# kisarur/minimap2-fpga

Measured on AMD Instinct MI355X. Metric: anchors/sec chained, higher is better.
Workload: dtype int32; 1 GPU; synthetic ONT anchor stream (mixed), 5000 anchors/read, map-ont chaining params (max_dist=5000, bw=500, max_iter=5000, max_skip=25), HBM-resident; reads_whole_batch=65536, distinct_reads=8192, anchors_per_read=5000, preset=map-ont, ragged=False, parallelism=read-sharded x1

## Files before the change

### include/mm2chain.h

```cpp
#ifndef MM2CHAIN_H
#define MM2CHAIN_H

#include <stdint.h>
#include <stddef.h>

#ifdef __cplusplus
extern "C" {
#endif

typedef struct { uint64_t x, y; } mm2c_anchor_t;

enum {
	MM2C_OK = 0,
	MM2C_E_NODEVICE = -1,
	MM2C_E_ARG = -2,
	MM2C_E_TOOBIG = -3,
	MM2C_E_HIP = -4
};

#define MM2C_F_IGNORE_SEG  0x1
#define MM2C_F_FORCE_GENERAL 0x2

typedef struct {
	int32_t max_dist_x, max_dist_y, bw;
// ... 13 lines not shown
int  mm2c_numa_cpulist(const char *sysfs_root, const char *pci_bus_id, char *buf, size_t len);
int  mm2c_slot_worker_node(int slot);
int  mm2c_split_tasks(int64_t n_tasks, const int64_t *offsets, int n_parts, int64_t *bounds );
void mm2c_shutdown(void);
const char *mm2c_last_error(void);
int  mm2c_device_info(char *name, size_t name_len, int *cu_count, size_t *hbm_bytes);
int  mm2c_device_identity(int *ordinal, char *pci_bus_id, size_t bus_len, char *arch, size_t arch_len);
int  mm2c_tune(const char *key, int value);

int  mm2c_split_model(const char *preset, float *k1_hw, float *k2_hw, float *c_hw, float *k_sw, float *c_sw);

void mm2c_params_map_ont(mm2c_params_t *p);
void mm2c_params_fpga_v2(mm2c_params_t *p, int32_t max_dist_x, int32_t max_dist_y, int32_t bw, int32_t q_span);

typedef struct mm2c_plan mm2c_plan_t;
mm2c_plan_t *mm2c_plan_create(const mm2c_params_t *par, int64_t n_tasks, const int64_t *h_offsets);
void mm2c_plan_destroy(mm2c_plan_t *plan);
int64_t mm2c_plan_total_anchors(const mm2c_plan_t *plan);

#define MM2C_STREAM_LIBRARY ((void *)(intptr_t)-1)

int mm2c_plan_run_device(mm2c_plan_t *plan, const void *d_anchors, const float *d_avg_qspan,
                         int32_t *d_f, int32_t *d_p, void *stream);

int mm2c_plan_set_device_offsets(mm2c_plan_t *plan, const int64_t *d_offsets);

int mm2c_plan_run_device_n(mm2c_plan_t *plan, const void *d_anchors, int64_t n_anchors, const float *d_avg_qspan, int64_t n_avg,
                           int32_t *d_f, int64_t n_f, int32_t *d_p, int64_t n_p, void *stream);

int mm2c_plan_last_kernel_ms(mm2c_plan_t *plan, float *ms);
int mm2c_plan_last_route(mm2c_plan_t *plan, int64_t *pieces, int64_t *one_wave_pieces, int64_t *coop_pieces);
int mm2c_route_pieces(int64_t pieces, int64_t longest, int64_t total);
int mm2c_plan_last_variant(mm2c_plan_t *plan, char *buf, size_t len);
int  mm2c_last_host_variant(char *buf, size_t len);
int  mm2c_debug_label_hits(unsigned long long *hits , int reset);
int mm2c_plan_last_prepass_ms(mm2c_plan_t *plan, float *ms);

int mm2c_plan_predict_device(mm2c_plan_t *plan, const void *d_anchors, uint8_t *d_num_subparts,
                             int64_t *d_total_subparts, int64_t *d_total_trip_count, void *stream);

int mm2c_chain_batch_host(const mm2c_params_t *par, int64_t n_tasks, const int64_t *h_offsets,
                          const mm2c_anchor_t *h_anchors, const float *h_avg_qspan ,
                          int32_t *h_f, int32_t *h_p);

void *mm2c_pinned_alloc(size_t bytes);
void  mm2c_pinned_free(void *ptr);

#define MM2C_MAX_TASK_ANCHORS ((int64_t)2147483582)

int mm2c_chain_task_host(const mm2c_params_t *par, int64_t n, const mm2c_anchor_t *a, float avg_qspan_scaled,
                         int32_t *f, int32_t *p, int tid);

int mm2c_chain_task_host_pred(const mm2c_params_t *par, int64_t n, const mm2c_anchor_t *a, float avg_qspan_scaled,
                              int32_t *f, int32_t *p, int tid, float hw_time_pred, float sw_time_pred);

typedef struct { int32_t device; int32_t reserved; uint64_t passes, calls, anchors, declined; } mm2c_slot_stats_t;
int mm2c_get_slot_stats(int slot, mm2c_slot_stats_t *out);
int mm2c_route_slot(int n_slots, const int64_t *outstanding, int tid);

#ifndef MM2C_NO_MM_CHAIN_DP_DECL
mm2c_anchor_t *mm_chain_dp(int max_dist_x, int max_dist_y, int bw, int max_skip, int max_iter, int min_cnt,
                           int min_sc, float gap_scale, int is_cdna, int n_segs, int64_t n, mm2c_anchor_t *a,
                           int *n_u_, uint64_t **_u, void *km, int tid);
#endif


// ... 164 lines not shown
```

### minimap2-fpga_amd/csrc/api_internal.h

```cpp
#ifndef MM2C_API_INTERNAL_H
#define MM2C_API_INTERNAL_H
#include <hip/hip_runtime.h>
#include <algorithm>
#include <atomic>
#include <chrono>
#include <condition_variable>
#include <cstdarg>
#include <cstdio>
#include <cstdlib>
#include <cstring>
#include <functional>
#include <thread>
#include <mutex>
#include <numeric>
#include <vector>
#include "mm2chain.h"
#include "chain_kernel.h"

namespace mm2c_api {

extern thread_local char g_err[512];
int fail(int code, const char *fmt, ...);

#define HIP_TRY(expr) do { hipError_t e_ = (expr); if (e_ != hipSuccess) \
	return ::mm2c_api::fail(MM2C_E_HIP, "%s failed: %s (%s:%d)", #expr, hipGetErrorString(e_), __FILE__, __LINE__); } while (0)

struct ThreadCtx;

struct Global {
	std::mutex mu;
	std::atomic<bool> ready{false};
	int device = -1;
	std::vector<int> devices;
	std::atomic<int64_t> multi_min_anchors{1 << 20};
	std::atomic<int> ring_class{3};
	std::atomic<int> far_thr10{7};
	std::atomic<int> noskip_loop{1};
	std::atomic<int> heap_sort{0};
	std::atomic<int> wide_pct{40};
	std::atomic<int> split_streams{1};
	std::atomic<int> compact_ring{1};
	std::atomic<int> q24_ring{1};
	std::atomic<int> force_tab{0};
	std::atomic<int> far_ring{1};
	std::atomic<int> epi_fused{1};
	std::atomic<size_t> combine_max_anchors{1u << 17};
	std::atomic<size_t> stage_max_anchors{1u << 21};
	std::atomic<int64_t> pipeline_chunk_anchors{20 << 20};
	std::atomic<int64_t> pipeline_pieces{8}, pipeline_min_chunk{4 << 20};
	std::atomic<int64_t> pipeline_taper{0};
	std::atomic<int64_t> cut_below_tasks{4096};
	std::atomic<int> seg_min{256};
	std::atomic<int> coop_waves{16};
	std::atomic<int64_t> coop_max_tasks{1024};
	std::atomic<int> single_launch{1};
	std::atomic<int> fuse_st{1};
	std::atomic<int> seg_prepass{1};
	std::atomic<int> coop_w8_above{256};
	std::atomic<int> pin_workers{1};
	std::atomic<int> decline_when_busy{0};
	std::atomic<int> direct_pass{1};
	std::atomic<size_t> direct_max_anchors{1u << 18};
	std::atomic<int> host_st{0};
	std::atomic<int> fused_out{1};
	std::atomic<int> pipe_coop_chunks{1};
	std::atomic<int> combiner_lanes{4};
	std::atomic<int> coop_plans{2};
	std::atomic<int> plan_cut{1};
	std::atomic<int> plan_cut_min{8192};
	hipStream_t stream = nullptr;
	std::vector<ThreadCtx *> thread_ctxs;
	std::atomic<uint64_t> tasks{0}, anchors{0}, launches{0}, segments{0}, host_call_ns{0}, passes{0};
	uint64_t epoch = 0;
};
// ... 50 lines not shown

struct ThreadCtx {
	int device = -1;
	WholeSlot whole[2];
	SeedSlot seed[2];
	hipStream_t st = nullptr, st2 = nullptr;
	hipStream_t st3 = nullptr, st_up = nullptr;
	std::vector<hipEvent_t> evs;
	hipEvent_t ev = nullptr;
	mm2c::LaunchInfo last_info = {};
	char *d_in = nullptr, *d_out = nullptr, *d_scratch = nullptr;
	char *h_in = nullptr, *h_out = nullptr;
	unsigned *h_flag = nullptr;
	unsigned seq = 0;
	unsigned *d_cnt = nullptr;
	size_t cap_in = 0, cap_out = 0, cap_scratch = 0, cap_hin = 0, cap_hout = 0;
	void release()
	{
		if (d_in) (void)hipFree(d_in); if (d_out) (void)hipFree(d_out); if (d_scratch) (void)hipFree(d_scratch);
		if (h_in) (void)hipHostFree(h_in); if (h_out) (void)hipHostFree(h_out); if (h_flag) (void)hipHostFree(h_flag); if (d_cnt) (void)hipFree(d_cnt);
		if (st) (void)hipStreamDestroy(st); if (st2) (void)hipStreamDestroy(st2); if (ev) (void)hipEventDestroy(ev);
		if (st3) (void)hipStreamDestroy(st3); if (st_up) (void)hipStreamDestroy(st_up);
		for (hipEvent_t e : evs) (void)hipEventDestroy(e);
		whole[0].release(); whole[1].release();
		seed[0].release(); seed[1].release();
		*this = ThreadCtx();
	}
};

inline void format_variant(const mm2c::LaunchInfo &I, char *buf, size_t len)
{
	if (I.tile && I.coop) snprintf(buf, len, "chain_dp_coop<W=%d,NX=%d,NF=%d,GS1=%d,FAR=%d,TAB=%d> loop=%s classes=0 cut=0 compact=0 coop=%d st=%s", I.coop, I.nx, I.nf, I.gs1,
	                               I.far_, I.tab, I.asm_loop ? "asm" : "c++", I.coop, I.fused_st ? "kernel" : "prepass");
	else if (I.tile) snprintf(buf, len, "chain_dp_tile<NX=%d,NF=%d,SKIP=%d,GEN=%d,GS1=%d,FAR=%d,TAB=%d> loop=%s classes=%d cut=%d compact=%d q24=%d", I.nx, I.nf, I.skip, I.gen, I.gs1,
	                     I.far_, I.tab, I.asm_loop ? "asm" : "c++", I.classes, I.cut, I.c16, I.q24);
	else snprintf(buf, len, "chain_dp_wave<R=%d,SKIP=%d,GEN=%d,GS1=%d,FAR=%d> loop=c++ classes=0 cut=%d", I.r, I.skip, I.gen, I.gs1, I.far_, I.cut);
}
void note_host_variant(const mm2c::LaunchInfo &I);

int get_thread_ctx(ThreadCtx **out);
int get_batch_ctx(ThreadCtx **out, std::unique_lock<std::mutex> &hold);
int cur_device();
int n_devices();
bool in_split_worker();
bool should_split(int64_t total_anchors);
int run_split(int64_t n_tasks, const int64_t *h_offsets, const std::function<int(int, int64_t, int64_t)> &fn);
hipError_t create_partner_stream(hipStream_t *st);
int grow_device(char **p, size_t *cap, size_t need);
int grow_pinned(char **p, size_t *cap, size_t need, bool gpu_addressed = false);
inline size_t align16(size_t x) { return (x + 15) & ~(size_t)15; }
struct Layout {
	size_t at = 0;
	size_t take(size_t bytes) { const size_t o = at; at = (at + bytes + 255) & ~(size_t)255; return o; }
};
int check_params(const mm2c_params_t *p);
mm2c::KParams to_kparams(const mm2c_params_t *p);
int check_offsets(int64_t n_tasks, const int64_t *off);
int build_order(int64_t n_tasks, const int64_t *off, std::vector<int32_t> &order);
size_t layout_epilogue(mm2c::EpiArgs &E, char *base, size_t tot, size_t nt, size_t sort_tmp);
int epilogue_debug_phases();
hipError_t dev_alloc(void **out, size_t bytes);
void dev_free(void *p);
void dev_free_synced(void *p);

struct DeviceScope {
	int prev = -1; bool changed = false; hipError_t err = hipSuccess;
	explicit DeviceScope(int dev)
	{
// ... 70 lines not shown
```

### minimap2-fpga_amd/csrc/chain_dp_coop.h

```cpp
#ifndef MM2C_CHAIN_DP_COOP_H
#define MM2C_CHAIN_DP_COOP_H
#include "chain_dp_tile.h"

#ifndef MM2C_COOP_PROBE
#define MM2C_COOP_PROBE 0
#endif

namespace mm2c {

#ifndef MM2C_COOP_FAR_TILES
#define MM2C_COOP_FAR_TILES 4
#endif
constexpr int COOP_FAR_TILES = MM2C_COOP_FAR_TILES;
constexpr int COOP_NX = 16, COOP_NF = 8;
constexpr int COOP_NEVER = 0x7fffffff;

#ifndef MM2C_COOP_PUSH2
#define MM2C_COOP_PUSH2 1
#endif
constexpr int COOP_NC = 32;
constexpr int COOP_ST_MAX = (2 * 64 * 64 * 4 + COOP_NC * 64 * 12) / 8;
template <int W> struct CoopLds { static constexpr int KEYS = 0, CNTS = 2 * 64 * 8, MASKS = CNTS + 2 * 64 * 4, PAIRS = MASKS + 2 * 2 * 64 * 8, CXQ = PAIRS + 2 * 64 * 64 * 4,
                                                       CF = CXQ + COOP_NC * 64 * 8, QCNT = CF + COOP_NC * 64 * 4, BYTES = QCNT + 16; };
static_assert(COOP_NC >= COOP_NX + COOP_FAR_TILES, "the candidate rings hold every tile phase A deals");
// ... 536 lines not shown
#pragma unroll 4
					for (int k = 0; k < 63; ++k) {
						const int row_k = s_pair[k * 64 + lane];
						const long long key64 = mk_key(row_k + rdlane((int)(acc >> 32), 63 - k), i0 + k);
						acc = (row_k != SENT && key64 > acc) ? key64 : acc;
					}
				}
				if (BALLOT(!rank_ok((int)(unsigned)acc)) == 0) { all_done = true; own_f = (int)(acc >> 32); own_p = (int)(unsigned)acc; }
				else acc = acc0;
			}
#endif
			int row = cnt > 0 ? s_pair[lane] : SENT;
			for (int k = all_done ? cnt : 0; k < cnt;) {
				const int L = 63 - k;
				if (tents >> L & 1) {
					const int row_k = row;
					if (k + 1 < cnt) row = s_pair[(k + 1) * 64 + lane];
					if (BALLOT(rank_ok((int)(unsigned)acc)) >> L & 1) {
#if MM2C_COOP_PROBE != 3 && MM2C_COOP_PROBE != 4
						if ((tents & (L > 0 ? ~0ull >> (64 - L) : 0ull)) != 0) {
							const long long key64 = mk_key(row_k + rdlane((int)(acc >> 32), L), i0 + k);
							acc = (row_k != SENT && key64 > acc) ? key64 : acc;
						}
#endif
						++k;
						continue;
					}
					tents &= ~(1ull << L);
					tw_l = lane == L ? tw_l & 0x7fffffff : tw_l;
				}
				flush(k);
				int k2 = k;
				if (ASM) {
#define MM2C_CALL(FN, LO0) FN<NX, NF>(i0, __builtin_amdgcn_readfirstlane(k), cnt, P.max_skip, avg, f, p, pbase, a, t, own_x, tx1_l, own_q, tq1_l, span_l, lo_c, \
                                 LO0, tw_l, own_f, own_p, addr0, addr0b, lomc_v, ownst, rl, mdqbw_v, X.bw_v, sent_v, 0, 0 MM2C_LC_ARG)
#ifdef MM2C_LABEL_COUNT
					int lc_v = 0;
#endif
					if (FAR && tile_far) k2 = TAB ? MM2C_CALL(scan_tile_asm_tab_far, lo_l) : MM2C_CALL(scan_tile_asm_cmp_far, lo_l);
					else k2 = TAB ? MM2C_CALL(scan_tile_asm_tab, lo_l) : MM2C_CALL(scan_tile_asm_cmp, lo_l);
#undef MM2C_CALL
					k2 = __builtin_amdgcn_readfirstlane(k2);
				}
				if (k2 == k) {
					const int i = i0 + k;
					const int xi = rdlane(own_x, L), qi = rdlane(own_q, L);
					const int span_i = rdlane(span_l, L);
					const int lo = rdlane(lo_l, L);
					Carry c = { span_i, -1, 0 };
					if (i - lo > 0) {
						X.xi1 = xi - 1; X.qi1 = qi - 1; X.span_i = span_i; X.span1_v = span_i - 1;
						mask_t eq_run = 0; bool dr0 = false;
						if (eq_prev != 0) {
							const mask_t r = eq_prev >> L;
							const int e = (int)__builtin_ctzll(~r);
							if (e > k) dr0 = true;
							else if (e > 0) eq_run = ((1ull << e) - 1) << (L + 1);
						}
						X.lo = lo; X.stamp = i + 1; X.s16 = 1 + k; X.s16_v = X.s16;
						X.far_mode = FAR && lo < stamp_lo;
						if (!dr0) scan_anchor<NX, NF, SKIP, GEN, GS1, FAR, TAB, false, false>(P, X, M, lane, i0, k, eq_run, own_x, own_q, own_g, own_f, own_p, addr0, c);
						else scan_anchor<NX, NF, SKIP, GEN, GS1, FAR, TAB, true, false>(P, X, M, lane, i0, k, 0, own_x, own_q, own_g, own_f, own_p, addr0, c);
					}
					write_lane2(own_f, own_p, __builtin_amdgcn_readfirstlane(c.best), __builtin_amdgcn_readfirstlane(c.best_j), L);
					k2 = k + 1;
				}
#if MM2C_COOP_PROBE != 3 && MM2C_COOP_PROBE != 4
// ... 51 lines not shown
```

### minimap2-fpga_amd/csrc/chain_dp_tile.h

```cpp
#ifndef MM2C_CHAIN_DP_TILE_H
#define MM2C_CHAIN_DP_TILE_H
#ifndef MM2C_DEEP_PREFETCH
#define MM2C_DEEP_PREFETCH 0
#endif
#include "chain_wave.h"

namespace mm2c {

__device__ __forceinline__ int usat_sub(int a, int b)
{
	int r;
	asm("v_sub_u32_e64 %0, %1, %2 clamp" : "=v"(r) : "v"(a), "v"(b));
	return r;
}
__device__ __forceinline__ int min3i(int a, int b, int c)
{
	int r;
	asm("v_min3_i32 %0, %1, %2, %3" : "=v"(r) : "v"(a), "v"(b), "v"(c));
	return r;
}
__device__ __forceinline__ int add3i(int a, int b, int c)
{
	int r;
	asm("v_add3_u32 %0, %1, %2, %3" : "=v"(r) : "v"(a), "v"(b), "v"(c));
	return r;
}
__device__ __forceinline__ void lds_store_b16_masked(mask_t m, int byte_addr, int value)
{
	asm volatile("s_mov_b64 exec, %0\n\tds_write_b8 %1, %2\n\ts_mov_b64 exec, -1" : : "s"(m), "v"(byte_addr), "v"(value) : "memory");
}
__device__ __forceinline__ void write_lane2(int &v0, int &v1, int a0, int a1, int l)
{
	asm("s_mov_b32 m0, %2\n\tv_writelane_b32 %0, %3, m0\n\tv_writelane_b32 %1, %4, m0"
	    : "+v"(v0), "+v"(v1) : "s"(l), "s"(a0), "s"(a1));
}

template <int NX, int NF, bool GEN, bool TAB, int RING = 0>
struct Lds {
	static constexpr int SN = 64 * NX;
	static constexpr int XS = RING ? 4 : 8;
	static constexpr int TILE = 64 * XS;
	static constexpr int RB = SN * XS;
	static constexpr int XQ = 0, FP = RB, ST = FP + NF * 512, QH = ST + SN, GAP = QH + (RING == 2 ? SN : 0),
	                     G = GAP + (TAB ? 1024 : 0), BYTES = G + (GEN ? NX * 64 : 0);
	static constexpr int FMASK = NF * 512 - 1;
	static constexpr int SBITS = __builtin_ctz(SN);
};

constexpr int FBIAS = 14;

struct AnchorCtx {
	int xi1, qi1;
	int span_i, seg_i;
	int lo;
	int stamp, s16;
	int stamp_lo;
	int far_mode;
	float avg;
	int mdq1_v, bw_v, span1_v, s16_v, rl;
};

struct TileMem {
	char *lds;
	const uint4 *a; const int32_t *f, *p; int32_t *t;
	int pbase;
};

template <bool GEN, bool FULL, bool DR0>
__device__ __forceinline__ mask_t chunk_filter(const KParams &P, const AnchorCtx &X, mask_t in_w, int dr1, int dq1, int dd, int gj, mask_t &same)
{
	mask_t valid;
	if (!GEN) {
		const int viol = usat_sub(dq1, X.mdq1_v) | usat_sub(dd, X.bw_v);
		valid = BALLOT(viol == 0);
		if (!FULL) valid &= in_w;
		if (DR0) valid &= BALLOT(dr1 != -1);
	} else {
		same = BALLOT(gj == X.seg_i);
		valid = pair_filter<true>(P, FULL ? ~0ull : in_w, dr1 + 1, dq1 + 1, dd, same);
	}
	return valid;
}

template <class LY, bool SKIP, bool GEN, bool GS1, bool FAR, bool TAB>
__device__ __forceinline__ bool chunk_finish(const KParams &P, const AnchorCtx &X, const TileMem &M, mask_t valid, mask_t same,
                                             int dr1, int dq1, int dd, int fj, int pj, int base, int lane, Carry &c)
{
	constexpr int SN = LY::SN;
	mask_t marked = 0;
	if (SKIP) {
		mask_t mk = valid & BALLOT(pj >= X.lo);
		if (FAR && X.far_mode) {
			const mask_t fm = mk & BALLOT(pj < X.stamp_lo);
			if (fm != 0) {
				int pj2 = pj;
				asm volatile("" : "+v"(pj2));
				if (fm >> lane & 1) __hip_atomic_store(&M.t[pj2], X.stamp, __ATOMIC_RELAXED, __HIP_MEMORY_SCOPE_WORKGROUP);
				mk &= ~fm;
			}
		}
		lds_store_b16_masked(mk, LY::ST + (pj & (SN - 1)), X.s16_v);
		const int tj = *(const uint8_t *)(M.lds + LY::ST + (X.rl + (base & (SN - 1))));
		marked = valid & BALLOT(tj == X.s16);
	}
	int sc;
	if (!GEN && TAB) {
		const int g = *(const int16_t *)(M.lds + LY::GAP + (min((unsigned)dd, 511u) << 1));
		sc = add3i(min3i(dq1, dr1, X.span1_v), fj, g);
	} else sc = pair_score<GEN, GS1>(P, X.avg, dr1 + 1, dq1 + 1, dd, same, X.span_i) + fj;
	const int scv = sel(valid, SENT, sc);
	return fold_lean<SKIP>(P, base + 63, marked, scv, c);
}

template <class LY, int NF>
__device__ __forceinline__ void ring_fp(const TileMem &M, int addr, int depth, int base, int rl, int &fj, int &pj)
{
	if (depth <= NF) {
		const int o = (LY::XS == 4 ? addr << 1 : addr) & LY::FMASK;
		const int2 fp = *(const int2 *)(M.lds + LY::FP + o);
		fj = fp.x + FBIAS; pj = fp.y;
	} else {
		const int j = max(base + rl, 0);
		fj = __hip_atomic_load(&M.f[j], __ATOMIC_RELAXED, __HIP_MEMORY_SCOPE_WORKGROUP);
		pj = __hip_atomic_load(&M.p[j], __ATOMIC_RELAXED, __HIP_MEMORY_SCOPE_WORKGROUP);
		pj = max(pj - M.pbase, -1);
	}
}

template <class LY, bool SKIP, bool GEN, bool GS1, bool TAB, bool DR0>
__device__ __forceinline__ bool far_chunk(const KParams &P, const AnchorCtx &X, const TileMem &M, mask_t in_w, int base, int lane, Carry &c)
{
	const int j = base + X.rl;
	int xj = 0, qj = 0, gj = 0;
	if (in_w >> lane & 1) {
		const uint4 aj = M.a[j];
		xj = (int)aj.x; qj = (int)aj.z;
		if (GEN) gj = (aj.w >> 16) & 0xff;
	}
	const int dr1 = X.xi1 - xj, dq1 = X.qi1 - qj;
	const int dd = absdiff(dr1, dq1);
	mask_t same = ~0ull;
	const mask_t valid = chunk_filter<GEN, false, DR0>(P, X, in_w, dr1, dq1, dd, gj, same);
	if (valid == 0) return false;
	int fj = 0, pj = -1;
	const bool vl = valid >> lane & 1;
	if (vl) {
		fj = __hip_atomic_load(&M.f[j], __ATOMIC_RELAXED, __HIP_MEMORY_SCOPE_WORKGROUP);
		pj = __hip_atomic_load(&M.p[j], __ATOMIC_RELAXED, __HIP_MEMORY_SCOPE_WORKGROUP);
		if (pj >= 0) pj -= M.pbase;
	}
// ... 97 lines not shown
#define MM2C_DPP_PREFIX_MAX(R) MM2C_DPP_STEP(R, "row_shr:1 row_mask:0xf bank_mask:0xf") MM2C_DPP_STEP(R, "row_shr:2 row_mask:0xf bank_mask:0xf") \
	MM2C_DPP_STEP(R, "row_shr:4 row_mask:0xf bank_mask:0xf") MM2C_DPP_STEP(R, "row_shr:8 row_mask:0xf bank_mask:0xf") \
	MM2C_DPP_STEP(R, "row_bcast:15 row_mask:0xa bank_mask:0xf") MM2C_DPP_STEP(R, "row_bcast:31 row_mask:0xc bank_mask:0xf")
#define MM2C_FILTER(X, Q) "v_sub_u32 %[dr], %[xi1], " X "\n\t" "v_sub_u32 %[dq], %[qi1], " Q "\n\t"
#define MM2C_FILTER2 "v_sub_u32_e64 %[u1], %[dq], %[mdqbw] clamp\n\t" "v_sad_u32 %[dd], %[dr], %[dq], 0\n\t" "v_max_u32 %[u1], %[u1], %[dd]\n\t" \
	"v_cmp_ge_u32 vcc, %[bw], %[u1]\n\t"
#define MM2C_R_XQ "v[62:63]"
#define MM2C_R_X "v62"
#define MM2C_R_Q "v63"
#define MM2C_R_FP "v[60:61]"
#define MM2C_R_F "v60"
#define MM2C_R_P "v61"
#define MM2C_XQ1_W "ds_read_b64 " MM2C_R_XQ ", %[addr1] offset:%[XQOFF]\n\t"
#define MM2C_XQ1_C "ds_read_b32 " MM2C_R_X ", %[addr1] offset:%[XQOFF]\n\t"
#define MM2C_BACK_W "v_add_u32 %[addr], 0xfffffe00, %[addr]\n\t" "v_and_b32 %[addr], %[RBM1], %[addr]\n\t"
#define MM2C_BACK_C "v_add_u32 %[addr], 0xffffff00, %[addr]\n\t" "v_and_b32 %[addr], %[RBM1], %[addr]\n\t"
#define MM2C_NEXT_XQ_W "ds_read_b64 " MM2C_R_XQ ", %[addr] offset:%[XQOFF]\n\t" MM2C_BACK_W
#define MM2C_NEXT_XQ_C "ds_read_b32 " MM2C_R_X ", %[addr] offset:%[XQOFF]\n\t" MM2C_BACK_C
#define MM2C_RFILTER_W MM2C_FILTER("" MM2C_R_X "", "" MM2C_R_Q "")
#define MM2C_OWNFILTER_W MM2C_FILTER("%[tx]", "%[tq]")
#define MM2C_FARFILTER_W MM2C_FILTER("%[fx]", "%[fq]")
#define MM2C_RDXQ_W "v_readfirstlane_b32 %[xi1], %[tx1]\n\t" "v_readfirstlane_b32 %[qi1], %[tq1]\n\t"
#define MM2C_SUB16(D, S0SEL, V, S1SEL) "v_sub_u16_sdwa " D ", %[xi1], " V " dst_sel:WORD_0 dst_unused:UNUSED_PAD src0_sel:" S0SEL " src1_sel:" S1SEL "\n\t"
#define MM2C_RFILTER_C MM2C_SUB16("%[dq]", "WORD_1", MM2C_R_X, "WORD_1") MM2C_SUB16("%[dr]", "WORD_0", MM2C_R_X, "WORD_0")
#define MM2C_OWNFILTER_C MM2C_SUB16("%[dq]", "WORD_1", "%[tx]", "WORD_1") MM2C_SUB16("%[dr]", "WORD_0", "%[tx]", "WORD_0")
#define MM2C_FARFILTER_C MM2C_SUB16("%[dq]", "WORD_1", "%[fq]", "WORD_0") MM2C_SUB16("%[dr]", "WORD_0", "%[fx]", "WORD_0")
#define MM2C_RDXQ_C "v_readfirstlane_b32 %[xi1], %[tx1]\n\t"
#define MM2C_XQ1_Q "ds_read_b32 " MM2C_R_X ", %[addr1] offset:%[XQOFF]\n\t" "ds_read_u8 " MM2C_R_Q ", %[addr1q] offset:%[QHOFF]\n\t"
#define MM2C_NEXT_XQ_Q "v_lshrrev_b32 %[u2], 2, %[addr]\n\t" "ds_read_b32 " MM2C_R_X ", %[addr] offset:%[XQOFF]\n\t" "ds_read_u8 " MM2C_R_Q ", %[u2] offset:%[QHOFF]\n\t" MM2C_BACK_C
#define MM2C_RFILTER_Q "v_sub_u16_sdwa %[dr], %[xi1], " MM2C_R_X " dst_sel:WORD_0 dst_unused:UNUSED_PAD src0_sel:WORD_0 src1_sel:WORD_0\n\t" \
	"v_perm_b32 %[u1], " MM2C_R_Q ", " MM2C_R_X ", %[selq]\n\t" "v_sub_u32 %[dq], %[qi1], %[u1]\n\t"
#define MM2C_OLDADDR_W "v_add_u32 %[vb], 0x400, %[addr]\n\t"
#define MM2C_OLDADDR_C "v_add_lshl_u32 %[vb], %[addr], %[c200], 1\n\t"
#define MM2C_FAR_REQ "v_add_u32 %[u2], %[fb], %[rl]\n\t" "v_max_i32 %[u2], 0, %[u2]\n\t" "v_lshlrev_b32 %[u2], 4, %[u2]\n\t" \
	"global_load_dword %[fx], %[u2], %[aptr]\n\t" "global_load_dword %[fq], %[u2], %[aptr] offset:8\n\t" "s_sub_i32 %[fb], %[fb], 64\n\t"
#define MM2C_SCORE_CMP "v_or_b32 %[va], 1, %[dd]\n\t" "v_ffbh_u32 %[va], %[va]\n\t" "v_lshrrev_b32 %[va], 1, %[va]\n\t" "v_cvt_f32_u32 %[vc], %[dd]\n\t" \
	"v_mul_f32 %[vc], %[avg], %[vc]\n\t" "v_cvt_i32_f32 %[vc], %[vc]\n\t" "v_min3_i32 %[sc], %[dq], %[dr], %[span1]\n\t" "v_sub_u32 %[sc], %[sc], %[vc]\n\t"
#define MM2C_ADDF_CMP "v_add3_u32 %[sc], %[sc], %[va], " MM2C_R_F "\n\t"
#define MM2C_SCORE_TAB "v_min_u32 %[va], 0x1ff, %[dd]\n\t" "v_lshlrev_b32 %[va], 1, %[va]\n\t" "ds_read_i16 %[va], %[va] offset:%[GAPOFF]\n\t" \
	"v_min3_i32 %[sc], %[dq], %[dr], %[span1]\n\t"
#define MM2C_ADDF_TAB "v_add3_u32 %[sc], %[sc], %[va], " MM2C_R_F "\n\t" "v_add_u32 %[sc], 14, %[sc]\n\t"

#define MM2C_DONE_FAR ""
#define MM2C_RD_FAR \
	"v_readfirstlane_b32 %[lo], %[tlo]\n\t" \
	"v_readfirstlane_b32 %[lo0], %[tlo0]\n\t"
#define MM2C_RD_LEAN ""
#define MM2C_LK_FAR \
	"s_sub_i32 %[fb], %[i0], %[REACH]\n\t" \
	"s_bitcmp1_b32 %[pk], 30\n\t" \
	"s_cbranch_scc0 Lnf_%=\n\t" \
	MM2C_FAR_REQ \
	"Lnf_%=:\n\t"
#define MM2C_LK_LEAN ""
#define MM2C_HF_FAR \
	"v_cmp_le_i32 vcc, %[lo], " MM2C_R_P "\n\t" \
	"s_and_b64 %[mk], vcc, %[valid]\n\t" \
	"v_and_b32 %[u2], %[SNM1], " MM2C_R_P "\n\t" \
	"s_mov_b64 exec, %[mk]\n\t" \
	"ds_write_b8 %[u2], %[s16v] offset:%[STOFF]\n\t" \
	"s_mov_b64 exec, %[valid]\n\t" \
	"ds_read_i8 %[vb], %[vb] offset:%[STOFF]\n\t" \
	"s_bitcmp1_b32 %[pk], 30\n\t" \
	"s_cbranch_scc0 Lmk_%=\n\t" \
	"v_cmp_le_i32 vcc, %[lo0], " MM2C_R_P "\n\t" \
	"s_andn2_b64 %[mask], vcc, %[mk]\n\t"       \
// ... 131 lines not shown
#define MM2C_PROBE_LK MM2C_P_X MM2C_P_X
#elif MM2C_PROBE == 11
#define MM2C_PROBE_LK "v_readlane_b32 %[t1], %[tw], %[c]\n\tv_readlane_b32 %[t0], %[tx], %[c]\n\tv_readlane_b32 %[last], %[tq], %[c]\n\tv_readlane_b32 %[base], %[tlo0], %[c]\n\t"
#elif MM2C_PROBE == 12
#define MM2C_PROBE_LK "s_mov_b32 m0, %[c]\n\ts_nop 0\n\tv_writelane_b32 %[u1], %[c], m0\n\tv_writelane_b32 %[u1], %[c], m0\n\t"
#elif MM2C_PROBE == 13
#define MM2C_P_X "s_branch 1f\n\ts_nop 0\n1:\n\t"
#define MM2C_PROBE_LK MM2C_P_X MM2C_P_X MM2C_P_X MM2C_P_X
#endif
#ifndef MM2C_PROBE_LK
#define MM2C_PROBE_LK ""
#endif
#ifndef MM2C_PROBE_OPERAND
#define MM2C_PROBE_OPERAND
#endif
#ifndef MM2C_PROBE_LOOP
#define MM2C_PROBE_LOOP ""
#endif
#define MM2C_R_F2 "v58"
#define MM2C_R_P2 "v59"
#define MM2C_FG_CLOB_PF0
#define MM2C_FG_CLOB_PF2 , MM2C_R_F2, MM2C_R_P2
#define MM2C_FG_CLOB(SEL) MM2C_FG_CLOB_##SEL
#define MM2C_FG_PLAIN(SCORE) \
	"s_lshl_b32 %[t0], %[d], 6\n\t" \
	"s_sub_i32 %[base], %[i0], %[t0]\n\t" \
	"v_add_u32 %[u2], %[base], %[rl]\n\t" \
	"v_max_i32 %[u2], 0, %[u2]\n\t" \
	"v_lshlrev_b32 %[u2], 2, %[u2]\n\t" \
	"global_load_dword " MM2C_R_P ", %[u2], %[pptr] sc0\n\t" \
	"global_load_dword " MM2C_R_F ", %[u2], %[fptr] sc0\n\t" \
	SCORE \
	"s_waitcnt vmcnt(0)\n\t"
#if MM2C_DEEP_PREFETCH
#define MM2C_FG_W(SCORE) \
	"s_lshl_b32 %[t0], %[d], 6\n\t" \
	"s_sub_i32 %[base], %[i0], %[t0]\n\t" \
	"s_cmp_eq_u32 %[base], %[bpre]\n\t" \
	"s_cbranch_scc1 Lfgh_%=\n\t" \
	"v_add_u32 %[u2], %[base], %[rl]\n\t" \
	"v_max_i32 %[u2], 0, %[u2]\n\t" \
	"v_lshlrev_b32 %[u2], 2, %[u2]\n\t" \
	"global_load_dword " MM2C_R_P ", %[u2], %[pptr] sc0\n\t" \
	"global_load_dword " MM2C_R_F ", %[u2], %[fptr] sc0\n\t" \
	SCORE \
	"s_waitcnt vmcnt(0)\n\t" \
	"s_branch Lfgp_%=\n" \
	"Lfgh_%=:\n\t" \
	SCORE \
	"s_waitcnt vmcnt(0)\n\t" \
	"v_mov_b32 " MM2C_R_P ", " MM2C_R_P2 "\n\t" \
	"v_mov_b32 " MM2C_R_F ", " MM2C_R_F2 "\n" \
	"Lfgp_%=:\n\t" \
	"s_or_b32 %[t0], %[n], %[part]\n\t"             \
	"s_cbranch_scc0 Lfgx_%=\n\t" \
	"s_sub_i32 %[bpre], %[base], 64\n\t" \
	"v_add_u32 %[u2], %[bpre], %[rl]\n\t" \
	"v_max_i32 %[u2], 0, %[u2]\n\t" \
	"v_lshlrev_b32 %[u2], 2, %[u2]\n\t" \
	"global_load_dword " MM2C_R_P2 ", %[u2], %[pptr] sc0\n\t" \
	"global_load_dword " MM2C_R_F2 ", %[u2], %[fptr] sc0\n" \
	"Lfgx_%=:\n\t"
#else
#define MM2C_FG_W(SCORE) MM2C_FG_PLAIN(SCORE)
#endif

// ... 12 lines not shown
#define MM2C_LC_OPERAND
#endif
#define MM2C_LB_K "0x1"
#define MM2C_LB_OWN "0x2"
#define MM2C_LB_LOOP "0x4"
#define MM2C_LB_OLD "0x8"
#define MM2C_LB_HF "0x10"
#define MM2C_LB_FARSTAMP "0x20"
#define MM2C_LB_BRKA "0x40"
#define MM2C_LB_FG "0x80"
#define MM2C_LB_PART "0x100"
#define MM2C_LB_PARTPASS "0x200"
#define MM2C_LB_IMP "0x400"
#define MM2C_LB_B0 "0x800"
#define MM2C_LB_SLOW2 "0x1000"
#define MM2C_LB_SLOW "0x2000"
#define MM2C_LB_B1 "0x4000"
#define MM2C_LB_B1M "0x8000"
#define MM2C_LB_B2 "0x10000"
#define MM2C_LB_B2CLOSED "0x20000"
#define MM2C_LB_LI "0x40000"
#define MM2C_LB_LICLOSED "0x80000"
#define MM2C_LB_CFB "0x100000"
#define MM2C_LB_GEN "0x200000"
#define MM2C_LB_BK "0x400000"
#define MM2C_LB_TK "0x800000"
#define MM2C_LB_AF "0x1000000"
#define MM2C_LB_END "0x2000000"
#define MM2C_LB_FLOOP "0x4000000"
#define MM2C_LB_FPART "0x8000000"
#define MM2C_LB_FOLD "0x10000000"
#define MM2C_LB_DONE "0x20000000"
#define MM2C_LB_SPEC "0x40000000"
#define MM2C_SCAN_TILE_ASM(NAME, TABV, C16V, XQ1, NEXT_XQ, RFILTER, OLDADDR, BACK, OWNFILTER, FARFILTER, RDXQ, SEG_FG, CLOB, SCORE, ADDF, SEG_RD, SEG_LK, SEG_HF, SEG_TAIL, SEG_END, SEG_DONE, LNEXT) \
template <int NX, int NF> \
__device__ __forceinline__ int NAME(int i0, int k_start, int cnt, int max_skip, float avg, const int32_t *f, const int32_t *p, int pbase, const uint4 *a, \
                                    int32_t *tg, int tx, int tx1, int tq, int tq1, int tspan, int tlo, int tlo0, int tw, int &own_f, int &own_p, \
                                    int addr1, int addr2, int lomc, int ownst, int rl, int mdqbw_v, int bw_v, int sent_v, int addr1q, int selq_v MM2C_LC_PARAM) \
{ \
	typedef Lds<NX, NF, false, TABV, C16V> LY; \
	typedef Lds<NX, NF, false, true, C16V> LYT; \
	int best, bestj, nskip, n, nfull, part, base, t0, t1, last, c, pk, lo, lo0, xi1, qi1, span1, s16, d, fb, bpre; \
	mask_t mask, valid, mk, marked, nm, se, ex, oh, pr; (void)pr; \
	int dr, dq, dd, u1, u2, sc, va, vb, vc, addr, s16v, lom1v, fx, fq; \
	asm volatile( \
		"s_mov_b64 %[ex], exec\n\t" \
		"s_mov_b32 %[bpre], 0x7fffffff\n\t"        \
		"s_sub_i32 %[c], %[kstart], %[cnt]\n\t"     \
		"s_sub_i32 %[t0], 63, %[kstart]\n\t" \
		"s_lshl_b64 %[mask], 1, %[t0]\n\t" \
		"s_lshr_b64 %[oh], %[mask], 1\n\t" \
		"s_or_b64 %[oh], %[oh], %[mask]\n\t"       \
		"s_mov_b64 exec, %[mask]\n\t" \
		MM2C_READ_ANCHOR(SEG_RD, RDXQ) \
		"s_mov_b64 exec, %[ex]\n" \
		"Lk_%=:\n\t" \
		MM2C_LC(MM2C_LB_K) \
		MM2C_PROBE_LK \
		"s_mov_b32 %[bestj], -1\n\t" \
		"s_cmp_lt_i32 %[pk], 0\n\t" \
		"s_cbranch_scc1 Lspec_%=\n\t"               \
		SEG_LK \
		"s_bfe_u32 %[n], %[pk], 0x40015\n\t"        \
		XQ1 \
		"v_mov_b32 %[addr], %[addr2]\n\t" \
		"s_add_i32 %[span1], %[best], -1\n\t" \
		"s_mov_b32 %[nskip], 0\n\t" \
		"s_bfe_u32 %[part], %[pk], 0x6000f\n\t"     \
		"s_mov_b32 %[nfull], %[n]\n\t" \
		"v_mov_b32 %[s16v], %[c]\n\t" \
		"s_and_b32 %[t0], %[pk], 63\n\t" \
		"s_cbranch_scc0 Lloop_%=\n\t" \
		"s_bfe_u32 %[t1], %[pk], 0x70008\n\t" \
		"s_bfm_b64 %[mask], %[t0], %[t1]\n\t" \
		OWNFILTER MM2C_FILTER2 \
		"s_and_b64 %[valid], vcc, %[mask]\n\t" \
		"s_cbranch_scc0 Lloop_%=\n\t" \
		MM2C_LC(MM2C_LB_OWN) \
		"s_mov_b32 %[d], 0\n\t" \
		"v_add_u32 " MM2C_R_F ", -14, %[own_f]\n\t" \
		"v_mov_b32 " MM2C_R_P ", %[own_p]\n\t" \
		"v_mov_b32 %[vb], %[ownst]\n\t" \
		SCORE \
		"s_branch Lhf_%=\n" \
		"Lloop_%=:\n\t" \
		MM2C_LC(MM2C_LB_LOOP) \
		MM2C_PROBE_LOOP \
		"s_sub_u32 %[n], %[n], 1\n\t" \
		"s_cbranch_scc1 Lpart_%=\n\t" \
		"s_waitcnt lgkmcnt(0)\n\t" \
		RFILTER NEXT_XQ MM2C_FILTER2 \
		"s_cbranch_vccz Lloop_%=\n\t" \
		"s_mov_b64 %[valid], vcc\n\t" \
		"s_sub_i32 %[d], %[nfull], %[n]\n" \
		"Lold_%=:\n\t" \
		MM2C_LC(MM2C_LB_OLD) \
		OLDADDR                                         \
		"v_and_b32 %[u2], %[FMASK], %[vb]\n\t"           \
		"v_bfe_u32 %[vb], %[vb], 3, %[SBITS]\n\t"        \
		"s_cmp_gt_u32 %[d], %[NFI]\n\t" \
		"s_cbranch_scc1 Lfg_%=\n\t" \
		"ds_read_b64 " MM2C_R_FP ", %[u2] offset:%[FPOFF]\n\t" \
		SCORE \
		"s_waitcnt lgkmcnt(0)\n" \
		"Lhf_%=:\n\t" \
		MM2C_LC(MM2C_LB_HF) \
		SEG_HF \
		"Lmk_%=:\n\t"                                   \
		"s_waitcnt lgkmcnt(0)\n\t" \
		"v_cmp_eq_u32 vcc, %[c], %[vb]\n" \
		"Lmk2_%=:\n\t" \
		ADDF \
		"s_and_b64 %[marked], vcc, exec\n\t" \
		"v_cmp_lt_i32 vcc, %[best], %[sc]\n\t" \
		"s_cbranch_vccnz Limp_%=\n\t" \
		"s_mov_b64 exec, %[ex]\n\t" \
		SEG_TAIL \
		"Lfg_%=:\n\t" \
		MM2C_LC(MM2C_LB_FG) \
		SEG_FG(SCORE) \
		"v_subrev_u32 " MM2C_R_P ", %[pbase], " MM2C_R_P "\n\t" \
		"v_max_i32 " MM2C_R_P ", -1, " MM2C_R_P "\n\t" \
		"v_add_u32 " MM2C_R_F ", -14, " MM2C_R_F "\n\t" \
		"s_branch Lhf_%=\n" \
		"Lpart_%=:\n\t" \
		MM2C_LC(MM2C_LB_PART) \
		"s_mov_b32 %[n], 0\n\t" \
		"s_cmp_eq_u32 %[part], 0\n\t" \
		"s_cbranch_scc1 Lend_%=\n\t" \
		"s_waitcnt lgkmcnt(0)\n\t" \
		RFILTER MM2C_FILTER2 \
		"s_sub_i32 %[t0], 64, %[part]\n\t" \
		"s_lshr_b64 %[mask], -1, %[t0]\n\t" \
		"s_mov_b32 %[part], 0\n\t" \
		"s_and_b64 %[valid], vcc, %[mask]\n\t" \
		"s_cbranch_scc0 Lend_%=\n\t" \
		MM2C_LC(MM2C_LB_PARTPASS) \
		"s_add_i32 %[d], %[nfull], 1\n\t" \
		BACK \
		"s_branch Lold_%=\n" \
		"Limp_%=:\n\t" \
		MM2C_LC(MM2C_LB_IMP) \
		"s_ff1_i32_b64 %[t0], %[valid]\n\t" \
		"v_readfirstlane_b32 %[t1], %[sc]\n\t"           \
		"s_cmp_gt_i32 %[t1], %[best]\n\t" \
		"s_cbranch_scc0 Lslow_%=\n\t" \
		"v_cmp_lt_i32 vcc, %[t1], %[sc]\n\t" \
		"s_cbranch_vccnz Lslow2_%=\n\t" \
		"s_mov_b64 exec, %[ex]\n\t" \
		MM2C_LC(MM2C_LB_B0) \
		"s_mov_b32 %[best], %[t1]\n\t" \
		"s_lshl_b32 %[t1], %[d], 6\n\t" \
		"s_sub_i32 %[bestj], %[i063], %[t1]\n\t"    \
		"s_sub_i32 %[bestj], %[bestj], %[t0]\n\t" \
		"s_sub_i32 %[nskip], %[nskip], 1\n\t" \
		"s_max_i32 %[nskip], %[nskip], 0\n\t" \
// ... 126 lines not shown
		"s_add_i32 %[t0], %[base], 63\n\t" \
		"s_sub_i32 %[bestj], %[t0], %[t1]\n" \
		"Laf_%=:\n\t" \
		MM2C_LC(MM2C_LB_AF) \
		"s_cmp_eq_u32 %[last], 63\n\t" \
		"s_cbranch_scc1 Lret_%=\n\t" \
		"s_branch Ldone_%=\n" \
		SEG_END(SCORE, FARFILTER) \
		"Ldone_%=:\n\t" \
		MM2C_LC(MM2C_LB_DONE) \
		SEG_DONE \
		"s_mov_b64 exec, %[oh]\n\t"                \
		"v_mov_b32 %[own_f], %[best]\n\t" \
		"v_mov_b32 %[own_p], %[bestj]\n\t" \
		MM2C_READ_ANCHOR(SEG_RD, RDXQ)                      \
		"s_mov_b64 exec, %[ex]\n\t" \
		"s_lshr_b64 %[oh], %[oh], 1\n\t" \
		"s_add_u32 %[c], %[c], 1\n\t"               \
		"s_cbranch_scc0 Lk_%=\n\t" \
		"s_branch Lexit_%=\n" \
		"Lspec_%=:\n\t" \
		MM2C_LC(MM2C_LB_SPEC) \
		"s_bitcmp1_b32 %[pk], 29\n\t" \
		"s_cbranch_scc1 Ldone_%=\n" \
		"Lexit_%=:\n\t" \
		"s_waitcnt vmcnt(0) lgkmcnt(0)\n\t" \
		: [best] "=&s"(best), [bestj] "=&s"(bestj), [nskip] "=&s"(nskip), [n] "=&s"(n), [nfull] "=&s"(nfull), [part] "=&s"(part), [base] "=&s"(base), \
		  [t0] "=&s"(t0), [t1] "=&s"(t1), [last] "=&s"(last), [c] "=&s"(c), [pk] "=&s"(pk), [lo] "=&s"(lo), [xi1] "=&s"(xi1), [qi1] "=&s"(qi1), \
		  [span1] "=&s"(span1), [s16] "=&s"(s16), [d] "=&s"(d), [lo0] "=&s"(lo0), [fb] "=&s"(fb), [bpre] "=&s"(bpre), \
		  [mask] "=&s"(mask), [valid] "=&s"(valid), [mk] "=&s"(mk), [marked] "=&s"(marked), [nm] "=&s"(nm), [se] "=&s"(se), [ex] "=&s"(ex), [oh] "=&s"(oh), \
		  [dr] "=&v"(dr), [dq] "=&v"(dq), [dd] "=&v"(dd), [u1] "=&v"(u1), [u2] "=&v"(u2), \
		  [sc] "=&v"(sc), [va] "=&v"(va), [vb] "=&v"(vb), [vc] "=&v"(vc), [addr] "=&v"(addr), [s16v] "=&v"(s16v), [lom1v] "=&v"(lom1v), [fx] "=&v"(fx), [fq] "=&v"(fq), \
		  [own_f] "+v"(own_f), [own_p] "+v"(own_p) MM2C_PROBE_OPERAND MM2C_LC_OPERAND \
		: [i0] "s"(i0), [kstart] "s"(k_start), [cnt] "s"(cnt), [icnt1] "s"(i0 + cnt + 1), [i063] "s"(i0 + 63), [c200] "s"(0x200), [maxskip] "s"(max_skip), [avg] "s"(avg), [fptr] "s"(f), [pptr] "s"(p), [pbase] "s"(pbase), [aptr] "s"(a), [tptr] "s"(tg), \
		  [tx] "v"(tx), [tx1] "v"(tx1), [tq] "v"(tq), [tq1] "v"(tq1), [tspan] "v"(tspan), [tlo] "v"(tlo), [tlo0] "v"(tlo0), [tw] "v"(tw), \
		  [addr1] "v"(addr1), [addr2] "v"(addr2), [lomc] "v"(lomc), [ownst] "v"(ownst), [rl] "v"(rl), [mdqbw] "v"(mdqbw_v), [bw] "v"(bw_v), [sent] "v"(sent_v), \
		  [addr1q] "v"(addr1q), [selq] "v"(selq_v), [QHOFF] "n"(LY::QH), \
		  [XQOFF] "n"(LY::XQ), [FPOFF] "n"(LY::FP), [STOFF] "n"(LY::ST), [RBM1] "n"(LY::RB - 1), [FMASK] "n"(LY::FMASK), \
		  [SNM1] "n"(LY::SN - 1), [RMASK] "n"(64 * NX - 1), [SBITS] "n"(LY::SBITS), [NFI] "n"(NF), [GAPOFF] "n"(LYT::GAP), [NXM1] "n"(NX - 1), [REACH] "n"(64 * NX) \
		: "memory", "vcc", "scc", MM2C_R_X, MM2C_R_Q, MM2C_R_F, MM2C_R_P MM2C_FG_CLOB(CLOB)); \
	return cnt + c; \
}

#define MM2C_RING_W MM2C_XQ1_W, MM2C_NEXT_XQ_W, MM2C_RFILTER_W, MM2C_OLDADDR_W, MM2C_BACK_W, MM2C_OWNFILTER_W, MM2C_FARFILTER_W, MM2C_RDXQ_W, MM2C_FG_W, PF2
#define MM2C_RING_C MM2C_XQ1_C, MM2C_NEXT_XQ_C, MM2C_RFILTER_C, MM2C_OLDADDR_C, MM2C_BACK_C, MM2C_OWNFILTER_C, MM2C_FARFILTER_C, MM2C_RDXQ_C, MM2C_FG_PLAIN, PF0
#define MM2C_SCAN_TILE_ASM_(...) MM2C_SCAN_TILE_ASM(__VA_ARGS__)
#define MM2C_LEAN MM2C_RD_LEAN, MM2C_LK_LEAN, MM2C_HF_LEAN, MM2C_TAIL_LEAN, MM2C_END_LEAN, "", "Lloop_%="
#define MM2C_FARS MM2C_RD_FAR, MM2C_LK_FAR, MM2C_HF_FAR, MM2C_TAIL_FAR, MM2C_END_FAR, MM2C_DONE_FAR, "Lret_%="
MM2C_SCAN_TILE_ASM_(scan_tile_asm_cmp, false, false, MM2C_RING_W, MM2C_SCORE_CMP, MM2C_ADDF_CMP, MM2C_LEAN)
MM2C_SCAN_TILE_ASM_(scan_tile_asm_tab, true, false, MM2C_RING_W, MM2C_SCORE_TAB, MM2C_ADDF_TAB, MM2C_LEAN)
MM2C_SCAN_TILE_ASM_(scan_tile_asm_cmp_far, false, false, MM2C_RING_W, MM2C_SCORE_CMP, MM2C_ADDF_CMP, MM2C_FARS)
MM2C_SCAN_TILE_ASM_(scan_tile_asm_tab_far, true, false, MM2C_RING_W, MM2C_SCORE_TAB, MM2C_ADDF_TAB, MM2C_FARS)
MM2C_SCAN_TILE_ASM_(scan_tile_asm_cmp_c, false, true, MM2C_RING_C, MM2C_SCORE_CMP, MM2C_ADDF_CMP, MM2C_LEAN)
MM2C_SCAN_TILE_ASM_(scan_tile_asm_tab_c, true, true, MM2C_RING_C, MM2C_SCORE_TAB, MM2C_ADDF_TAB, MM2C_LEAN)
MM2C_SCAN_TILE_ASM_(scan_tile_asm_cmp_far_c, false, true, MM2C_RING_C, MM2C_SCORE_CMP, MM2C_ADDF_CMP, MM2C_FARS)
MM2C_SCAN_TILE_ASM_(scan_tile_asm_tab_far_c, true, true, MM2C_RING_C, MM2C_SCORE_TAB, MM2C_ADDF_TAB, MM2C_FARS)
#define MM2C_RING_Q MM2C_XQ1_Q, MM2C_NEXT_XQ_Q, MM2C_RFILTER_Q, MM2C_OLDADDR_C, MM2C_BACK_C, MM2C_OWNFILTER_W, MM2C_FARFILTER_W, MM2C_RDXQ_W, MM2C_FG_PLAIN, PF0
MM2C_SCAN_TILE_ASM_(scan_tile_asm_cmp_q, false, 2, MM2C_RING_Q, MM2C_SCORE_CMP, MM2C_ADDF_CMP, MM2C_LEAN)
MM2C_SCAN_TILE_ASM_(scan_tile_asm_tab_q, true, 2, MM2C_RING_Q, MM2C_SCORE_TAB, MM2C_ADDF_TAB, MM2C_LEAN)
MM2C_SCAN_TILE_ASM_(scan_tile_asm_cmp_far_q, false, 2, MM2C_RING_Q, MM2C_SCORE_CMP, MM2C_ADDF_CMP, MM2C_FARS)
MM2C_SCAN_TILE_ASM_(scan_tile_asm_tab_far_q, true, 2, MM2C_RING_Q, MM2C_SCORE_TAB, MM2C_ADDF_TAB, MM2C_FARS)

template <int NX, int NF, bool SKIP, bool GEN, bool GS1, bool FAR, bool TAB, int C16 >
#ifdef MM2C_LABEL_COUNT
#define MM2C_WAVES_PER_SIMD(C16V, BYTES) 1
#else
#define MM2C_WAVES_PER_SIMD(C16V, BYTES) ((C16V) == 1 && (BYTES) <= 6144 ? 7 : (C16V) == 2 && (BYTES) <= 7424 ? 6 : 1)
#endif
__global__ void __launch_bounds__(64, MM2C_WAVES_PER_SIMD(C16, (Lds<NX, NF, GEN, TAB, C16>::BYTES)))
chain_dp_tile(KParams P, int64_t n_tasks, const int64_t *__restrict__ offsets, const int32_t *__restrict__ order,
              const uint4 *__restrict__ a_all, const float *__restrict__ avg_in, const int32_t *__restrict__ pbase_in,
              const int32_t *__restrict__ st_all, int32_t *__restrict__ f_all, int32_t *__restrict__ p_all, int32_t *__restrict__ t_all,
              int32_t *__restrict__ status, int only_flagged, const int64_t *__restrict__ ends, const int32_t *__restrict__ n_live,
              const uint8_t *__restrict__ cls, int my_cls, int cls_mask)
{
	static_assert(!C16 || (SKIP && !GEN && (GS1 || TAB)), "the compact and the q24 ring belong to the variants of the hand-written loop");
	static_assert(NF >= 1 && NF < NX && (NF & (NF - 1)) == 0 && (NX & (NX - 1)) == 0, "rings of a power of two of tiles, addressed with masks");
	static_assert(NF <= NX, "the f / p ring holds a prefix of the tiles of the x / q ring");
	static_assert(64 * (NX - 1) < 1024, "bef (anchors of older tiles inside the ring window) travels in the 10-bit field bits 15-24 of the per-anchor word");
	typedef Lds<NX, NF, GEN, TAB, C16> LY;
	constexpr int SN = LY::SN;
	constexpr bool ASMV = SKIP && !GEN && (GS1 || TAB);
	const bool ASM = ASMV && P.bw >= 0 && P.max_dq - 1 >= P.bw;
	__shared__ __attribute__((aligned(16))) char lds[LY::BYTES];

	const int lane = threadIdx.x;
	const int64_t task = order ? (int64_t)__builtin_amdgcn_readfirstlane(order[blockIdx.x]) : (int64_t)blockIdx.x;
	if (task >= n_tasks) return;
	if (n_live && task >= (int64_t)*n_live) return;
	if (only_flagged && status[task] == 0) return;
	if (cls && (cls[task] & cls_mask) != my_cls) return;
	const int64_t base0 = offsets[task];
	const int n = __builtin_amdgcn_readfirstlane((int)((ends ? ends[task] : offsets[task + 1]) - base0));
	if (n <= 0) return;
	const uint4 *a = a_all + base0;
	const int32_t *st = st_all + base0;
	int32_t *f = f_all + base0, *p = p_all + base0, *t = FAR ? t_all + base0 : nullptr;
	if (ASMV && (uint32_t)(uintptr_t)(void *)lds != 0) { if (lane == 0) status[task] = 3; return; }

	const int pbase = pbase_in ? pbase_in[task] : 0;
	const int st_sub = ends ? pbase : 0;

	float avg = avg_in ? avg_in[task] : -1.0f;
	if (avg < 0.f) {
		uint64_t sum = 0;
		for (int k = lane; k < n; k += 64) sum += (a[k].w & 0xffu);
		for (int o = 32; o > 0; o >>= 1) sum += __shfl_xor(sum, o);
		avg = (float)(__dmul_rn(.01, (double)(float)sum) / (double)n);
	}
	avg = __builtin_bit_cast(float, __builtin_amdgcn_readfirstlane(__builtin_bit_cast(int, avg)));
	if (TAB) {
		int16_t *const s_gap = (int16_t *)(lds + LY::GAP);
		for (int dd = lane; dd <= P.bw && dd < 512; dd += 64) {
			const int lg = dd ? 31 - __builtin_clz((unsigned)dd) : 0;
			int g = (int)((float)dd * avg) + (lg >> 1);
			if (P.gap_scale != 1.0f) g = (int)__dadd_rn(__dmul_rn((double)g, (double)P.gap_scale), .499);
			s_gap[dd] = (int16_t)(1 - g);
		}
	}

	const int rl = 63 - lane;
	AnchorCtx X;
	X.avg = avg; X.rl = rl; X.seg_i = 0; X.far_mode = 0;
	X.mdq1_v = P.max_dq - 1; X.bw_v = P.bw;
	int sent_v = SENT, mdqbw_v = P.max_dq - 1 - P.bw;
	int selq_v = 0x0c040302;
	asm volatile("" : "+v"(X.mdq1_v), "+v"(X.bw_v), "+v"(sent_v), "+v"(mdqbw_v));
	if (C16 == 2) asm volatile("" : "+v"(selq_v));
	TileMem M;
	M.lds = lds; M.a = a; M.f = f; M.p = p; M.t = t; M.pbase = pbase;

	int own_x = 0, own_q = 0, own_g = 0, own_f = 0, own_p = -1;
	int seg0 = 0;
	bool t_ready = false;
	const bool no_pairs = !GEN && (P.max_dq <= 0 || P.bw < 0);

#ifdef MM2C_LABEL_COUNT
	int lc_v = 0;
#endif
	uint4 cur = (rl < n) ? a[rl] : make_uint4(0, 0, 0, 0);
	int cur_st = (rl < n) ? st[rl] - st_sub : 0;
	for (int i0 = 0; i0 < n; i0 += 64) {
		const int idx = i0 + rl;
		const int cnt = __builtin_amdgcn_readfirstlane(min(64, n - i0));
		uint4 nxt = make_uint4(0, 0, 0, 0); int nxt_st = 0;
		if (idx + 64 < n) { nxt = a[idx + 64]; nxt_st = st[idx + 64] - st_sub; }
		int prev_last = rdlane(own_x, 0);
		own_x = (int)cur.x; own_q = (int)cur.z;
		own_g = (cur.w >> 16) & 0xff;
		const int own_xq = (int)(((unsigned)own_x & 0xffffu) | ((unsigned)own_q << 16));
		const int own_xq1 = (int)(((unsigned)(own_x - 1) & 0xffffu) | ((unsigned)(own_q - 1) << 16));
		(void)own_xq; (void)own_xq1;
		if (!GEN && !(P.flags & KF_IGNORE_SEG)) {
			if (i0 == 0) seg0 = rdlane(own_g, 63);
			if (BALLOT(rl < cnt && own_g != seg0)) { if (lane == 0) status[task] = 1; return; }
		}
		for (int s = lane; s < SN / 4; s += 64) ((int *)(lds + LY::ST))[s] = 0;
		const int stamp_lo = i0 - 64 * (NX - 1);
		{
			const int o = (idx & (SN - 1)) * LY::XS;
			if (C16) *(int *)(lds + LY::XQ + o) = own_xq;
			else *(int2 *)(lds + LY::XQ + o) = make_int2(own_x, own_q);
			if (C16 == 2) *(uint8_t *)(lds + LY::QH + (idx & (SN - 1))) = (uint8_t)((unsigned)own_q >> 16);
// ... 6 lines not shown
				t_ready = true;
			}
			if (t_ready && idx < n) t[idx] = 0;
		}
		const int span_l = P.span_override >= 0 ? P.span_override : (int)(cur.w & 0xff);
		mask_t eq_prev = 0;
		if (!GEN) {
			asm volatile("" : "+v"(prev_last));
			const int px = __builtin_amdgcn_update_dpp(prev_last, own_x, 0x130 , 0xf, 0xf, false);
			eq_prev = BALLOT(px == own_x);
			if (i0 == 0) eq_prev &= ~(1ull << 63);
		}
		X.stamp_lo = stamp_lo;
		const int addr0 = ((idx - 64) & (SN - 1)) * LY::XS;
		const int addr0b = ((idx - 128) & (SN - 1)) * LY::XS;
		int lomc_v = stamp_lo - 1;
		asm volatile("" : "+v"(lomc_v));

		const int lo_l = no_pairs ? idx : min(cur_st, idx);
		const mask_t above = ~(eq_prev >> lane);
		const int e_l = above ? (int)__builtin_ctzll(above) : 64;
		const int w_l = min(rl, idx - lo_l);
		const int lo_c = max(lo_l, stamp_lo), bef_l = max(i0 - lo_c, 0);
		int tw_l = max(w_l - e_l, 0) | (min(lane + 1 + e_l, 64) << 8) | (bef_l << 15);
		if (lo_l >= idx) tw_l |= (int)0xa0000000;
		if (FAR && lo_l < stamp_lo) tw_l |= 1 << 30;
		if (e_l > rl) tw_l |= (int)0x80000000;
		const bool tile_far = FAR && BALLOT((tw_l >> 30) & 1) != 0;
		const int ownst = idx & (SN - 1);
		const int tx1_l = own_x - 1, tq1_l = own_q - 1;

		for (int k = 0; k < cnt; ++k) {
			if (ASM) {
#define MM2C_CALL(FN, LO0) FN<NX, NF>(i0, __builtin_amdgcn_readfirstlane(k), cnt, P.max_skip, avg, f, p, pbase, a, t, own_x, tx1_l, own_q, tq1_l, span_l, lo_c, \
                                 LO0, tw_l, own_f, own_p, addr0, addr0b, lomc_v, ownst, rl, mdqbw_v, X.bw_v, sent_v, addr0 >> 2, selq_v MM2C_LC_ARG)
				if (C16 == 2) {
					if (FAR && tile_far) k = TAB ? MM2C_CALL(scan_tile_asm_tab_far_q, lo_l) : MM2C_CALL(scan_tile_asm_cmp_far_q, lo_l);
					else k = TAB ? MM2C_CALL(scan_tile_asm_tab_q, lo_l) : MM2C_CALL(scan_tile_asm_cmp_q, lo_l);
				} else if (C16) {
#define MM2C_CALLC(FN, LO0) FN<NX, NF>(i0, __builtin_amdgcn_readfirstlane(k), cnt, P.max_skip, avg, f, p, pbase, a, t, own_xq, own_xq1, own_xq, own_xq1, span_l, lo_c, \
                                 LO0, tw_l, own_f, own_p, addr0, addr0b, lomc_v, ownst, rl, mdqbw_v, X.bw_v, sent_v, 0, 0 MM2C_LC_ARG)
					if (FAR && tile_far) k = TAB ? MM2C_CALLC(scan_tile_asm_tab_far_c, lo_l) : MM2C_CALLC(scan_tile_asm_cmp_far_c, lo_l);
					else k = TAB ? MM2C_CALLC(scan_tile_asm_tab_c, lo_l) : MM2C_CALLC(scan_tile_asm_cmp_c, lo_l);
#undef MM2C_CALLC
				} else if (FAR && tile_far) k = TAB ? MM2C_CALL(scan_tile_asm_tab_far, lo_l) : MM2C_CALL(scan_tile_asm_cmp_far, lo_l);
				else k = TAB ? MM2C_CALL(scan_tile_asm_tab, lo_l) : MM2C_CALL(scan_tile_asm_cmp, lo_l);
#undef MM2C_CALL
#ifdef MM2C_LABEL_COUNT
				{
					const int row = (C16 == 1 ? 4 : 0) | (TAB ? 2 : 0) | ((FAR && tile_far) ? 1 : 0);
					if (lane < 32 && lc_v != 0) atomicAdd(&g_label_hits[row * 32 + lane], (unsigned long long)(unsigned)lc_v);
					lc_v = 0;
				}
#endif
				k = __builtin_amdgcn_readfirstlane(k);
				if (k >= cnt) break;
			}
			const int L = 63 - k;
			const int i = i0 + k;
			const int xi = rdlane(own_x, L), qi = rdlane(own_q, L);
			const int span_i = rdlane(span_l, L);
			const int lo = rdlane(lo_l, L);
			Carry c = { span_i, -1, 0 };
			if (i - lo > 0) {
				mask_t eq_run = 0; bool dr0 = false;
				if (!GEN && eq_prev != 0) {
					const mask_t r = eq_prev >> L;
					const int e = (int)__builtin_ctzll(~r);
					if (e > k) dr0 = true;
					else if (e > 0) eq_run = ((1ull << e) - 1) << (L + 1);
				}
				X.xi1 = xi - 1; X.qi1 = qi - 1; X.span_i = span_i; X.span1_v = span_i - 1;
				if (GEN) X.seg_i = rdlane(own_g, L);
				X.lo = lo; X.stamp = i + 1; X.s16 = 1 + k; X.s16_v = X.s16;
				X.far_mode = FAR && lo < stamp_lo;
				if (!dr0) scan_anchor<NX, NF, SKIP, GEN, GS1, FAR, TAB, false, C16>(P, X, M, lane, i0, k, eq_run, own_x, own_q, own_g, own_f, own_p, addr0, c);
				else scan_anchor<NX, NF, SKIP, GEN, GS1, FAR, TAB, true, C16>(P, X, M, lane, i0, k, 0, own_x, own_q, own_g, own_f, own_p, addr0, c);
			}
			write_lane2(own_f, own_p, __builtin_amdgcn_readfirstlane(c.best), __builtin_amdgcn_readfirstlane(c.best_j), L);
		}
		if (rl < cnt) { f[idx] = own_f; p[idx] = own_p < 0 ? own_p : own_p + pbase; }
		{
			const int o = (idx << 3) & LY::FMASK;
			*(int2 *)(lds + LY::FP + o) = make_int2(own_f - FBIAS, own_p);
		}
		cur = nxt; cur_st = nxt_st;
	}
}

}
#endif
```

### minimap2-fpga_amd/csrc/chain_kernel.h

```cpp
#ifndef MM2C_CHAIN_KERNEL_H
#define MM2C_CHAIN_KERNEL_H
#include <hip/hip_runtime.h>
#include <stdint.h>

namespace mm2c {

enum { KF_IGNORE_SEG = 0x1, KF_FORCE_GENERAL = 0x2 };
constexpr int CLS_STAT_SLOTS = 64;

struct KParams {
	int32_t max_dist_x, max_dist_y, bw;
	int32_t max_skip, max_iter;
	int32_t is_cdna, n_segs;
	int32_t span_override;
	int32_t max_dq;
	int32_t flags;
	float gap_scale;
};

struct CutArgs {
	int64_t max_pieces = 0;
	int32_t seg_min = 256;
	int32_t min_anchors = 8192;
	int64_t *d_start = nullptr, *d_end = nullptr;
	int32_t *d_pbase = nullptr, *d_status = nullptr, *d_count = nullptr;
	int32_t w8_above = 256;
	int32_t *d_live = nullptr;
	int32_t *d_has_cut = nullptr;
	float *d_avg = nullptr;
	uint8_t *d_cls = nullptr;
};

struct LaunchArgs {
	KParams P;
	int64_t n_tasks;
	const int64_t *d_offsets;
	const int32_t *d_order;
	const void *d_anchors;
	const float *d_avg;
	float *d_avg_ws = nullptr;
	uint8_t *d_cls = nullptr;
	hipStream_t side = nullptr;
	hipEvent_t ev_fork = nullptr, ev_join = nullptr;
	int noskip_loop = 1;
	int compact = 1;
	int q24 = 1;
	unsigned long long *d_cls_stat = nullptr;
	int wide_pct = 40;
	int far_thr10 = 7;
	int far_ring = 0;
	const int32_t *d_pbase;
	int32_t *d_f, *d_p;
	int32_t *d_t;
	int32_t *d_st;
	int32_t *d_status;
	int64_t max_task_anchors = 0;
	int64_t longest_task = 0;
	unsigned long long *d_seg_ws = nullptr;
	int coop_waves = 0;
	int dry_run = 0;
	const int64_t *hm_off = nullptr; const float *hm_avg = nullptr; const int32_t *hm_pbase = nullptr;
	const void *h_anchors = nullptr;
	int fuse_st = 1;
	int coop_w8_above = 256;
	int32_t *h_f = nullptr, *h_p = nullptr; unsigned *d_done = nullptr, *h_flag = nullptr; unsigned seq = 0;
	int st_ready = 0;
	int force_tab = 0;
	int ring_class;
	CutArgs cut;
};

struct LaunchInfo {
	int tile;
	int nx, nf, r;
	int skip, gen, gs1, far_, tab;
	int asm_loop;
	int classes;
	int c16;
	int q24;
	int cut;
	int coop;
	int host_out;
	int single_ok;
	int fused_st;
	int route_auto;
};
constexpr int COOP_ROUTE_MAX_PIECES = 2048;
__host__ __device__ inline bool coop_pays(long long n_pieces, long long longest, long long total, long long w8_above = 256)
{
	if (n_pieces <= 0 || n_pieces > COOP_ROUTE_MAX_PIECES) return false;
	return 1450ll * longest > total || (n_pieces > w8_above && longest >= 8192 && 2300ll * longest > total);
}


int chain_ring_anchors(int ring_class);
hipError_t label_hits_read(unsigned long long *out , bool reset);
hipError_t launch_predict(int32_t max_dist_x, int64_t n_tasks, const int64_t *d_offsets, const int32_t *d_order, const void *d_anchors,
                          uint8_t *d_num_subparts, int64_t *d_total_subparts, int64_t *d_total_trip, hipStream_t st);
hipError_t launch_chain_dp(const LaunchArgs &L, hipStream_t st, int *n_launches, hipEvent_t ev_dp_begin, LaunchInfo *info = nullptr);

}

#include "chain_aux.h"
#endif
```

### minimap2-fpga_amd/csrc/chain_kernel.hip

```cpp

#include <hip/hip_runtime.h>
#include <cstdlib>
#include <algorithm>
#include <stdint.h>
#include <limits.h>
#include <stdlib.h>
#include "chain_kernel.h"
#include "chain_wave.h"
#ifndef MM2C_NX
#define MM2C_NX 8
#define MM2C_NF 2
#endif
#ifndef MM2C_NF1
#define MM2C_NF1 2
#endif
#ifndef MM2C_CNX
#define MM2C_CNX 16
#endif
#ifndef MM2C_CNF
#define MM2C_CNF 2
#endif
#include "chain_dp_tile.h"
#include "chain_dp_coop.h"

namespace mm2c {

template <int R, bool FAR>
__device__ __forceinline__ int stamp_and_fetch(mask_t valid, int pj, int lo, int stamp_lo, int stamp, int s16_v, char *t_bytes,
                                               int32_t *t_glob, int lane, int own_off2)
{
	const mask_t mk = valid & BALLOT(pj >= lo);
	const int sink = ((stamp - 1) & (2 * R - 1)) << 1;
	int tgt = sel(mk, sink, (pj & (2 * R - 1)) << 1);
	if (FAR) {
		const mask_t fm = mk & BALLOT(pj < stamp_lo);
		if (fm != 0) {
			int pj2 = pj;
			asm volatile("" : "+v"(pj2));
			if (fm >> lane & 1) __hip_atomic_store(&t_glob[pj2], stamp, __ATOMIC_RELAXED, __HIP_MEMORY_SCOPE_WORKGROUP);
			tgt = sel(fm, tgt, sink);
		}
	}
	*(uint16_t *)(t_bytes + tgt) = (uint16_t)s16_v;
	__builtin_amdgcn_fence(__ATOMIC_RELEASE, "wavefront");
	__builtin_amdgcn_wave_barrier();
	return *(const uint16_t *)(t_bytes + own_off2);
}

struct Win { int x, q, f, p, g; };
#define NV 3
// ... 103 lines not shown
			const int dd = absdiff(dr, dq);
			const mask_t same = GEN ? BALLOT(wg == seg_i) : ~0ull;
			const mask_t valid = pair_filter<GEN>(P, first_lanes(rem), dr, dq, dd, same);
			if (valid != 0) {
				int tj = 0;
				if (SKIP) tj = stamp_and_fetch<R, FAR>(valid, wp, lo, stamp_lo, stamp, s16_v, t_bytes, t, lane,
				                                        (((jtop << 1) + nl2) & ((2 * R - 1) << 1)));
				const int sc = pair_score<GEN, GS1>(P, avg, dr, dq, dd, same, span_i) + wf;
				const int scv = sel(valid, SENT, sc);
				const mask_t marked = SKIP ? BALLOT(tj == s16) : 0;
				broke = fold_chunk<SKIP, false>(P, jtop, valid, marked, scv, c);
			}
			jtop -= 64; rem -= 64;
		}
		if (broke) return;
		for (; rem >= 64; jtop -= 64, rem -= 64)
			if (older_chunk<R, SKIP, GEN, GS1, FAR, true>(P, avg, lane, i, lo, lds_lo, stamp_lo, stamp, s16, s16_v, xi, qi, span_i, seg_i, jtop, rem,
			                                              vt, xq_bytes, fp_bytes, s_g, t_bytes, s_t, a, f, p, t, pbase, c)) return;
		if (rem > 0)
			older_chunk<R, SKIP, GEN, GS1, FAR, false>(P, avg, lane, i, lo, lds_lo, stamp_lo, stamp, s16, s16_v, xi, qi, span_i, seg_i, jtop, rem,
			                                           vt, xq_bytes, fp_bytes, s_g, t_bytes, s_t, a, f, p, t, pbase, c);
	}
}

constexpr int PREPASS_SEG = 32768;
template <bool SEG>
__global__ void __launch_bounds__(256)
chain_window_start_t(KParams P, int64_t n_tasks, const int64_t *__restrict__ offsets, const int32_t *__restrict__ order,
                   const ulonglong2 *__restrict__ a_all, int32_t *__restrict__ st_all, int32_t *__restrict__ has_cut ,
                   float *__restrict__ avg_out , uint8_t *__restrict__ cls_out , int far_ring, int far_thr10,
                   unsigned long long *__restrict__ cls_stat ,
                   unsigned q_span_max ,
                   int q24 ,
                   int seg_anchors, unsigned long long *__restrict__ seg_ws)
{
	const int lane = threadIdx.x;
	const int64_t task = order ? (int64_t)order[blockIdx.x] : (int64_t)blockIdx.x;
	if (task >= n_tasks) return;
	const int64_t base = offsets[task];
	const int n = (int)(offsets[task + 1] - base);
	const int s0 = SEG ? (int)min((long long)blockIdx.y * seg_anchors, (long long)INT_MAX) : 0;
	if (SEG && s0 >= n) return;
	const int s1 = SEG ? (int)min((long long)s0 + seg_anchors, (long long)n) : n;
	const ulonglong2 *a = a_all + base;
	int32_t *st = st_all + base;
	const uint64_t D = (uint64_t)(int64_t)P.max_dist_x;
	constexpr int RING = 2048;
	__shared__ uint64_t s_x[RING];
	__shared__ int s_prev;
	__shared__ unsigned long long s_sum;
	__shared__ unsigned long long s_far;
	__shared__ int s_qmin, s_qmax;
	if (lane == 0) { s_prev = 0; s_sum = 0; s_far = 0; s_qmin = INT_MAX; s_qmax = INT_MIN; }
	int q_min = INT_MAX, q_max = INT_MIN;
	const int max_dq = min(P.max_dist_x, P.max_dist_y);
	uint64_t far_sum = 0;
	uint64_t span_sum = 0;
	ulonglong2 nxt = s0 + lane < n ? a[s0 + lane] : make_ulonglong2(0, 0);
	for (int i0 = s0; i0 < s1; i0 += 256) {
		const int i = i0 + lane, cnt = min(256, n - i0);
		const ulonglong2 cur = nxt;
		if (i < n) { s_x[i & (RING - 1)] = cur.x; span_sum += (cur.y >> 32) & 0xff; q_min = min(q_min, (int)(uint32_t)cur.y); q_max = max(q_max, (int)(uint32_t)cur.y); }
		__syncthreads();
		if (i + 256 < n) nxt = a[i + 256];
		const int range_lo = max(s_prev, max(i0 - P.max_iter, 0)), len = i0 + cnt - range_lo;
		int lo = 0;
// ... 26 lines not shown
					const int dr = xi - xj, dq = qi - qj, dd = dr > dq ? dr - dq : dq - dr;
					chain |= (lane & 63) >= d && i - d >= lo && dr > 0 && dq > 0 && dq <= max_dq && dd <= P.bw;
				}
				if (beyond > 0 && !chain) far_sum += (uint64_t)((beyond + 63) >> 6);
			}
		}
		__syncthreads();
		if (i < n && lane == cnt - 1) s_prev = lo;
	}
	if constexpr (SEG) {
		for (int o = 32; o > 0; o >>= 1) { q_min = min(q_min, __shfl_xor(q_min, o)); q_max = max(q_max, __shfl_xor(q_max, o)); far_sum += __shfl_xor(far_sum, o); span_sum += __shfl_xor(span_sum, o); }
		if ((lane & 63) == 0) { atomicMin(&s_qmin, q_min); atomicMax(&s_qmax, q_max); if (far_sum) atomicAdd(&s_far, (unsigned long long)far_sum); atomicAdd(&s_sum, (unsigned long long)span_sum); }
		__syncthreads();
		__shared__ int s_last;
		unsigned long long *ws = seg_ws + 4 * task;
		if (lane == 0) {
			atomicAdd(&ws[0], s_sum); if (s_far) atomicAdd(&ws[1], s_far);
			atomicMax((unsigned *)&ws[2], ~((unsigned)s_qmin ^ 0x80000000u)); atomicMax((unsigned *)&ws[2] + 1, (unsigned)s_qmax ^ 0x80000000u);
			__threadfence();
			const unsigned n_seg = (unsigned)(((long long)n + seg_anchors - 1) / seg_anchors);
			const bool last = atomicAdd((unsigned *)&ws[3], 1u) == n_seg - 1;
			s_last = last;
			if (last) {
				__threadfence();
				s_sum = atomicAdd(&ws[0], 0ull); s_far = atomicAdd(&ws[1], 0ull);
				s_qmin = (int)(~atomicMax((unsigned *)&ws[2], 0u) ^ 0x80000000u); s_qmax = (int)(atomicMax((unsigned *)&ws[2] + 1, 0u) ^ 0x80000000u);
				ws[0] = 0; ws[1] = 0; ws[2] = 0; ws[3] = 0;
			}
		}
		__syncthreads();
		if (!s_last) return;
		far_sum = 0; span_sum = 0; q_min = s_qmin; q_max = s_qmax;
	}
	if (cls_out && n > 0) {
		for (int o = 32; o > 0; o >>= 1) { q_min = min(q_min, __shfl_xor(q_min, o)); q_max = max(q_max, __shfl_xor(q_max, o)); }
		if ((lane & 63) == 0) { atomicMin(&s_qmin, q_min); atomicMax(&s_qmax, q_max); }
		__syncthreads();
		const int wide = (q_span_max == 0 || (unsigned)s_qmax - (unsigned)s_qmin > q_span_max) ? 2 : 0;
		const int huge = (q24 && (s_qmin < 0 || s_qmax >= (1 << 24))) ? 4 : 0;
		if (far_ring == 1) {
			for (int o = 32; o > 0; o >>= 1) far_sum += __shfl_xor(far_sum, o);
			if ((lane & 63) == 0 && far_sum) atomicAdd(&s_far, (unsigned long long)far_sum);
			__syncthreads();
			if (lane == 0) {
				const int c = (!huge && n >= 1024 && 10 * s_far > (unsigned long long)far_thr10 * (unsigned long long)n) ? 1 : 0;
				cls_out[task] = (uint8_t)(c | wide | huge);
				if (cls_stat) {
					unsigned long long *cs = cls_stat + 4 * (task & (CLS_STAT_SLOTS - 1));
					atomicAdd(&cs[1], (unsigned long long)n); if (c) atomicAdd(&cs[0], (unsigned long long)n);
					if (wide) atomicAdd(&cs[3], (unsigned long long)n);
				}
			}
		} else if (lane == 0) {
			cls_out[task] = (uint8_t)((far_ring == 2 && !huge ? 1 : 0) | wide | huge);
			if (cls_stat) { unsigned long long *cs = cls_stat + 4 * (task & (CLS_STAT_SLOTS - 1)); atomicAdd(&cs[1], (unsigned long long)n); if (wide) atomicAdd(&cs[3], (unsigned long long)n); }
		}
	}
	if (avg_out && n > 0) {
		for (int o = 32; o > 0; o >>= 1) span_sum += __shfl_xor(span_sum, o);
		if ((lane & 63) == 0) atomicAdd(&s_sum, (unsigned long long)span_sum);
		__syncthreads();
		if (lane == 0) avg_out[task] = (float)(__dmul_rn(.01, (double)(float)s_sum) / (double)n);
	}
}

__global__ void __launch_bounds__(256)
chain_window_start_wide(KParams P, int64_t n_tasks, const int64_t *__restrict__ offsets, const ulonglong2 *__restrict__ a_all, int32_t *__restrict__ st_all,
                        unsigned *__restrict__ span_sum)
{
	const int64_t task = (int64_t)blockIdx.x;
	if (task >= n_tasks) return;
	const int64_t base = offsets[task];
	const int n = (int)(offsets[task + 1] - base);
	if ((int)blockIdx.y * 256 >= n) return;
	const int i = (int)blockIdx.y * 256 + (int)threadIdx.x;
	const ulonglong2 *a = a_all + base;
	if (span_sum) {
		unsigned v = i < n ? (unsigned)(a[i].y >> 32) & 0xffu : 0u;
		for (int o = 32; o > 0; o >>= 1) v += __shfl_xor(v, o);
		if ((threadIdx.x & 63) == 0 && v) atomicAdd(&span_sum[task], v);
	}
	if (i >= n) return;
	const uint64_t D = (uint64_t)(int64_t)P.max_dist_x;
	const uint64_t xi = a[i].x;
	int hi = i, lo = max(i - P.max_iter, 0);
	while (lo < hi) {
		const int mid = (lo + hi) >> 1;
		if (xi > a[mid].x + D) lo = mid + 1; else hi = mid;
	}
	st_all[base + i] = lo;
}

__global__ void __launch_bounds__(256)
// ... 11 lines not shown
	__syncthreads();
	if (threadIdx.x == 0) {
		const bool coop = coop_pays(n, s_max, (long long)s_tot, C.w8_above);
		const bool eight = n > C.w8_above;
		C.d_count[1] = coop ? 0 : n; C.d_count[2] = coop && !eight ? n : 0; C.d_count[3] = coop && eight ? n : 0;
	}
}

__global__ void __launch_bounds__(256)
chain_avg_finish(int64_t n_tasks, const int64_t *__restrict__ offsets, unsigned *__restrict__ sum_avg)
{
	const int64_t t = (int64_t)blockIdx.x * 256 + threadIdx.x;
	if (t >= n_tasks) return;
	const int64_t n = offsets[t + 1] - offsets[t];
	const unsigned sum = sum_avg[t];
	((float *)sum_avg)[t] = n > 0 ? (float)(__dmul_rn(.01, (double)(float)sum) / (double)n) : 0.f;
}

__global__ void __launch_bounds__(256)
chain_cls_settle(int64_t n_tasks, uint8_t *__restrict__ cls, const unsigned long long *__restrict__ cls_stat, int settle_ring, int wide_pct)
{
	__shared__ unsigned long long s_tot[4];
	if (threadIdx.x < 4) s_tot[threadIdx.x] = 0;
	__syncthreads();
	if (threadIdx.x < 4 * CLS_STAT_SLOTS) atomicAdd(&s_tot[threadIdx.x & 3], cls_stat[threadIdx.x]);
	__syncthreads();
	const int64_t t = (int64_t)blockIdx.x * 256 + threadIdx.x;
	if (t >= n_tasks) return;
	const bool all_wide = 100 * s_tot[3] > (unsigned long long)wide_pct * s_tot[1];
	const unsigned long long far = s_tot[0], all = s_tot[1];
	int c = cls[t];
	if (all_wide) c |= 2;
	if (settle_ring) {
		if (4 * far < all) c &= 6;
		else if (4 * far > 3 * all && !(c & 4)) c |= 1;
	}
	cls[t] = (uint8_t)c;
}

__global__ void __launch_bounds__(64)
chain_predict(int32_t max_dist_x, int64_t n_tasks, const int64_t *__restrict__ offsets, const int32_t *__restrict__ order,
              const ulonglong2 *__restrict__ a_all, uint8_t *__restrict__ nsub_all, int64_t *__restrict__ total_sub,
              int64_t *__restrict__ total_trip)
{
	const int lane = threadIdx.x;
	const int64_t task = order ? (int64_t)order[blockIdx.x] : (int64_t)blockIdx.x;
	if (task >= n_tasks) return;
	const int64_t base = offsets[task];
	const int n = (int)(offsets[task + 1] - base);
	const ulonglong2 *a = a_all + base;
	const uint64_t D = (uint64_t)(int64_t)max_dist_x;
	int64_t s_sub = 0, s_trip = 0;
	for (int i = lane; i < n; i += 64) {
		const uint64_t xi = a[i].x;
		int lo = 0, hi = i;
		while (lo < hi) {
			const int mid = (lo + hi) >> 1;
			if (xi > a[mid].x + D) lo = mid + 1; else hi = mid;
		}
		const int trip = min(i - lo, 1024);
		const int sub = trip / 128 + ((trip == 0 || trip % 128 > 0) ? 1 : 0);
		if (nsub_all) nsub_all[base + i] = (uint8_t)sub;
		s_sub += sub; s_trip += trip;
	}
	for (int o = 32; o > 0; o >>= 1) { s_sub += __shfl_xor(s_sub, o); s_trip += __shfl_xor(s_trip, o); }
	if (lane == 0) { if (total_sub) total_sub[task] = s_sub; if (total_trip) total_trip[task] = s_trip; }
}
// ... 159 lines not shown
		}
		if (lane < cnt) {
			const int o = i0 + cnt - 1 - lane;
			s_xq[o & (R - 1)] = make_uint2((uint32_t)wx, (uint32_t)wq);
			s_fp[o & (R - 1)] = make_int2(wf, wp);
			if (GEN) s_g[o & (R - 1)] = (uint8_t)wg;
			f[o] = wf; p[o] = wp < 0 ? wp : wp + pbase;
		}
		cur = nxt; cur_st = nxt_st;
	}
}

template <int R, bool SKIP, bool GEN, bool GS1, bool FAR>
static hipError_t launch_one(const LaunchArgs &L, hipStream_t st, int only_flagged)
{
	if (L.cut.max_pieces > 0) {
		hipLaunchKernelGGL((chain_dp_wave<R, SKIP, GEN, GS1, FAR>), dim3((unsigned)L.cut.max_pieces), dim3(64), 0, st,
		                   L.P, L.cut.max_pieces, L.cut.d_start, (const int32_t *)nullptr, (const uint4 *)L.d_anchors, L.cut.d_avg, L.cut.d_pbase, L.d_st, L.d_f, L.d_p,
		                   L.d_t, L.cut.d_status, only_flagged, L.cut.d_end, L.cut.d_count);
		return hipGetLastError();
	}
	hipLaunchKernelGGL((chain_dp_wave<R, SKIP, GEN, GS1, FAR>), dim3((unsigned)L.n_tasks), dim3(64), 0, st,
	                   L.P, L.n_tasks, L.d_offsets, L.d_order, (const uint4 *)L.d_anchors, L.d_avg, L.d_pbase, L.d_st, L.d_f, L.d_p, L.d_t,
	                   L.d_status, only_flagged, (const int64_t *)nullptr, (const int32_t *)nullptr);
	return hipGetLastError();
}

template <int NX, int NF, bool SKIP, bool GEN, bool GS1, bool FAR, bool TAB, int C16>
static hipError_t launch_tile_nx(const LaunchArgs &L, const float *d_avg, hipStream_t st, int only_flagged, bool with_cls, int my_cls, int cls_mask)
{
	if (L.cut.max_pieces > 0) {
		hipLaunchKernelGGL((chain_dp_tile<NX, NF, SKIP, GEN, GS1, FAR, TAB, C16>), dim3((unsigned)L.cut.max_pieces), dim3(64), 0, st,
		                   L.P, L.cut.max_pieces, L.cut.d_start, (const int32_t *)nullptr, (const uint4 *)L.d_anchors, L.cut.d_avg, L.cut.d_pbase, L.d_st, L.d_f, L.d_p,
		                   L.d_t, L.cut.d_status, only_flagged, L.cut.d_end, L.cut.d_live ? L.cut.d_live : L.cut.d_count, with_cls ? (const uint8_t *)L.cut.d_cls : (const uint8_t *)nullptr, my_cls, cls_mask);
		return hipGetLastError();
	}
	hipLaunchKernelGGL((chain_dp_tile<NX, NF, SKIP, GEN, GS1, FAR, TAB, C16>), dim3((unsigned)L.n_tasks), dim3(64), 0, st,
	                   L.P, L.n_tasks, L.d_offsets, L.d_order, (const uint4 *)L.d_anchors, d_avg, L.d_pbase, L.d_st, L.d_f, L.d_p, L.d_t,
	                   L.d_status, only_flagged, (const int64_t *)nullptr, (const int32_t *)nullptr, with_cls ? (const uint8_t *)L.d_cls : (const uint8_t *)nullptr, my_cls, cls_mask);
	return hipGetLastError();
}

static bool have_cls(const LaunchArgs &L) { return L.d_cls != nullptr && (L.cut.max_pieces == 0 || L.cut.d_cls != nullptr); }
static bool use_classes(const LaunchArgs &L, bool skip, bool gen) { return !gen && skip && L.far_ring != 0 && have_cls(L); }
static unsigned compact_q_span(const LaunchArgs &L, bool asm_loop)
{
	const KParams &P = L.P;
	if (!L.compact || !asm_loop || !have_cls(L) || P.max_dist_x < 0 || P.max_dist_x > 65535 || P.max_dq < 1 || P.max_dq > 32768) return 0;
	return 65535u - (unsigned)P.max_dq;
}

static bool q24_ring(const LaunchArgs &L, bool skip, bool gen, bool gs1, bool tab)
{
	return L.q24 != 0 && use_classes(L, skip, gen) && (gs1 || tab) && L.P.max_dist_x >= 0 && L.P.max_dist_x <= 65535;
}

template <bool SKIP, bool GEN, bool GS1, bool FAR, bool TAB>
static hipError_t launch_tile_one(const LaunchArgs &L, const float *d_avg, hipStream_t st, int only_flagged, int *n_launches)
{
	const bool classes = use_classes(L, SKIP, GEN);
	bool c16 = false;
	if constexpr (SKIP && !GEN && (GS1 || TAB)) c16 = compact_q_span(L, L.P.bw >= 0 && L.P.max_dq - 1 >= L.P.bw) != 0;
	const int wide = c16 ? 2 : 0, mask = (c16 ? 2 : 0) | (classes ? 1 : 0);
	const bool fork = c16 && L.side != nullptr && L.ev_fork != nullptr && L.ev_join != nullptr;
	hipStream_t sw = fork ? L.side : st;
	hipError_t e = hipSuccess;
	bool forked = false;
	if (fork) { e = hipEventRecord(L.ev_fork, st); if (e == hipSuccess) { e = hipStreamWaitEvent(sw, L.ev_fork, 0); forked = e == hipSuccess; } }
	if (e == hipSuccess) e = launch_tile_nx<MM2C_NX, MM2C_NF, SKIP, GEN, GS1, FAR, TAB, 0>(L, d_avg, sw, only_flagged, mask != 0, wide, mask);
	if constexpr (!GEN && SKIP)
		if (e == hipSuccess && classes) {
			bool done = false;
			if constexpr (GS1 || TAB)
				if (q24_ring(L, SKIP, GEN, GS1, TAB)) { e = launch_tile_nx<2 * MM2C_NX, MM2C_NF1, SKIP, GEN, GS1, FAR, TAB, 2>(L, d_avg, sw, only_flagged, true, wide | 1, mask); done = true; }
			if (!done) e = launch_tile_nx<2 * MM2C_NX, MM2C_NF1, SKIP, GEN, GS1, FAR, TAB, 0>(L, d_avg, sw, only_flagged, true, wide | 1, mask);
			if (n_launches) ++*n_launches;
		}
	bool joined = false;
	if (forked) joined = hipEventRecord(L.ev_join, sw) == hipSuccess;
	if constexpr (SKIP && !GEN && (GS1 || TAB))
		if (e == hipSuccess && c16) { e = launch_tile_nx<MM2C_CNX, MM2C_CNF, SKIP, GEN, GS1, FAR, TAB, 1>(L, d_avg, st, only_flagged, true, 0, 2); if (n_launches) ++*n_launches; }
	if (forked) {
		const hipError_t ej = joined ? hipStreamWaitEvent(st, L.ev_join, 0) : hipStreamSynchronize(sw);
		if (e == hipSuccess) e = joined ? ej : hipErrorUnknown;
	}
	return e;
}

template <int W>
static hipError_t launch_coop_w(const LaunchArgs &L, const float *d_avg, hipStream_t st, bool tab, int only_flagged, const int32_t *n_live, int32_t *st_out = nullptr, float *avg_out = nullptr, const uint4 *a_src = nullptr)
{
	const bool far_ = (int64_t)L.P.max_iter > 64 * (COOP_NX - 1);
	const dim3 block(64 * W);
	if (L.cut.max_pieces > 0) {
		const dim3 grid((unsigned)std::min<int64_t>(L.cut.max_pieces, COOP_ROUTE_MAX_PIECES));
#define MM2C_COOP(GS1, FAR, TAB) hipLaunchKernelGGL((chain_dp_coop<W, GS1, FAR, TAB>), grid, block, 0, st, L.P, L.cut.max_pieces, L.cut.d_start, (const int32_t *)nullptr, \
	                                            (const uint4 *)L.d_anchors, (const float *)L.cut.d_avg, L.cut.d_pbase, L.d_st, L.d_f, L.d_p, L.d_t, L.cut.d_status, only_flagged, \
	                                            (const int64_t *)L.cut.d_end, n_live, CoopHostOut(), (int32_t *)nullptr, (float *)nullptr, (const uint4 *)nullptr, CoopMeta())
		if (tab) { if (far_) MM2C_COOP(true, true, true); else MM2C_COOP(true, false, true); }
		else { if (far_) MM2C_COOP(true, true, false); else MM2C_COOP(true, false, false); }
#undef MM2C_COOP
		return hipGetLastError();
	}
	const dim3 grid((unsigned)L.n_tasks);
	CoopHostOut H;
	if (L.h_flag && L.h_f && L.h_p && L.d_done && (L.P.flags & KF_IGNORE_SEG) && !only_flagged) { H.f = L.h_f; H.p = L.h_p; H.d_done = L.d_done; H.h_flag = L.h_flag; H.seq = L.seq; }
	CoopMeta MT;
	if (a_src && H.h_flag && L.hm_off && L.hm_avg && L.hm_pbase && L.n_tasks <= COOP_META_MAX && !L.d_order) {
		MT.n = (int32_t)L.n_tasks;
		for (int64_t k = 0; k < L.n_tasks; ++k) { MT.off[k] = L.hm_off[k]; MT.avg[k] = L.hm_avg[k]; MT.pbase[k] = L.hm_pbase[k]; }
		MT.off[L.n_tasks] = L.hm_off[L.n_tasks];
	}
#define MM2C_COOP(GS1, FAR, TAB) hipLaunchKernelGGL((chain_dp_coop<W, GS1, FAR, TAB>), grid, block, 0, st, L.P, L.n_tasks, L.d_offsets, L.d_order, (const uint4 *)L.d_anchors, \
	                                            d_avg, L.d_pbase, L.d_st, L.d_f, L.d_p, L.d_t, L.d_status, only_flagged, (const int64_t *)nullptr, (const int32_t *)nullptr, H, st_out, avg_out, H.h_flag ? a_src : (const uint4 *)nullptr, MT)
// ... 86 lines not shown
	LaunchArgs L = L_in;
	const bool want_gen = L.P.is_cdna || L.P.n_segs > 1 || (L.P.flags & KF_FORCE_GENERAL);
	const bool loop_ok = L.P.gap_scale == 1.0f || L_in.force_tab || (L.P.bw <= 511 && L.P.gap_scale > -20.f && L.P.gap_scale < 20.f);
	if (L.noskip_loop && (int64_t)L.P.max_skip >= (int64_t)L.P.max_iter && L.P.max_iter >= 1 && L.ring_class >= 3 && !want_gen && L.P.bw >= 0 && L.P.max_dq - 1 >= L.P.bw && loop_ok)
		L.P.max_skip = L.P.max_iter - 1;
	const KParams &P = L.P;
	const bool skip = (int64_t)P.max_skip < (int64_t)P.max_iter;
	const bool gs1 = P.gap_scale == 1.0f;
	const int R = chain_ring_anchors(L.ring_class);
	const bool tile = L.ring_class >= 3;
	const bool tile_gen = L.ring_class >= 4;
	const bool far_ = (int64_t)P.max_iter > (int64_t)R;
	const bool far_old = (int64_t)P.max_iter > 256;
	static const bool force_tab_env = getenv("MM2C_FORCE_TAB") != nullptr;
	const bool force_tab = force_tab_env || L.force_tab != 0;
	const bool tab = tile && (!gs1 || force_tab) && P.bw >= 0 && P.bw <= 511 && P.gap_scale > -20.f && P.gap_scale < 20.f;
	const bool coop_cfg = tile && !want_gen && skip && (gs1 || tab) && P.bw >= 0 && P.max_dq - 1 >= P.bw;
	const bool coop = L.coop_waves > 1 && coop_cfg && L.cut.max_pieces == 0;
	const bool coop_auto = L.coop_waves < 0 && coop_cfg && L.cut.max_pieces > 0 && L.cut.d_count != nullptr;
	if (coop_auto) { L.cut.d_live = L.cut.d_count + 1; L.cut.w8_above = L.coop_w8_above; }
	if (info) {
		info->route_auto = coop_auto ? 1 : 0;
		info->fused_st = coop && coop_makes_st(L) ? 1 : 0;
		info->host_out = (coop && L.h_flag && L.h_f && L.h_p && L.d_done && (L.P.flags & KF_IGNORE_SEG)) ? 1 : 0;
		info->single_ok = info->fused_st && info->host_out && L.d_avg != nullptr;
		const bool t0 = tile && (!want_gen || tile_gen);
		info->coop = coop ? coop_width(L) : 0;
		info->tile = t0; info->nx = t0 ? MM2C_NX : 0; info->nf = t0 ? MM2C_NF : 0; info->r = t0 ? 64 * (MM2C_NX - 1) : (tile ? 256 : R);
		info->skip = skip; info->gen = want_gen; info->gs1 = gs1; info->far_ = t0 ? far_ : (tile ? far_old : far_); info->tab = t0 && tab && !want_gen;
		info->asm_loop = t0 && skip && !want_gen && (gs1 || tab) && P.bw >= 0 && P.max_dq - 1 >= P.bw;
		info->classes = t0 && use_classes(L, skip, want_gen);
		info->c16 = t0 && compact_q_span(L, info->asm_loop != 0) != 0;
		info->q24 = t0 && info->classes && q24_ring(L, skip, want_gen, gs1, tab);
		info->cut = L.cut.max_pieces > 0;
		if (coop) { info->nx = COOP_NX; info->nf = COOP_NF; info->r = 64 * (COOP_NX - 1); info->far_ = (int64_t)P.max_iter > 64 * (COOP_NX - 1); info->classes = 0; info->c16 = 0; info->q24 = 0; }
	}
	if (L.dry_run) return hipSuccess;
	float *avg_out = L.d_avg ? nullptr : L.d_avg_ws;
	const float *d_avg = L.d_avg ? L.d_avg : L.d_avg_ws;
	const unsigned c16_bound = tile && (!want_gen || tile_gen) ? compact_q_span(L, skip && !want_gen && (gs1 || tab) && P.bw >= 0 && P.max_dq - 1 >= P.bw) : 0u;
	const bool wide_prepass = coop && L.max_task_anchors > 0 && L.max_task_anchors <= (1 << 22) && (L.d_avg != nullptr || L.d_avg_ws != nullptr) && L.cut.max_pieces == 0
	                          && (L.max_task_anchors + 255) / 256 <= 65535;
	const bool no_prepass = coop && ((L.st_ready && L.d_avg != nullptr) || coop_makes_st(L));
	if (no_prepass) {
	} else if (wide_prepass) {
		unsigned *sums = L.d_avg ? nullptr : (unsigned *)L.d_avg_ws;
		if (sums && hipMemsetAsync(sums, 0, (size_t)L.n_tasks * 4, st) != hipSuccess) return hipGetLastError();
		hipLaunchKernelGGL(chain_window_start_wide, dim3((unsigned)L.n_tasks, (unsigned)((L.max_task_anchors + 255) / 256)), dim3(256), 0, st, P, L.n_tasks, L.d_offsets,
		                   (const ulonglong2 *)L.d_anchors, L.d_st, sums);
		if (sums) hipLaunchKernelGGL(chain_avg_finish, dim3((unsigned)((L.n_tasks + 255) / 256)), dim3(256), 0, st, L.n_tasks, L.d_offsets, sums);
	} else {
		const bool seg = L.d_seg_ws != nullptr && L.n_tasks <= 512 && L.longest_task >= 2 * PREPASS_SEG && (L.longest_task + PREPASS_SEG - 1) / PREPASS_SEG <= 65535;
#define MM2C_WS(SEG, GRID, SEGN, WS) hipLaunchKernelGGL(chain_window_start_t<SEG>, GRID, dim3(256), 0, st, P, L.n_tasks, L.d_offsets, L.d_order, \
	                   (const ulonglong2 *)L.d_anchors, L.d_st, L.cut.max_pieces > 0 ? L.cut.d_has_cut : (int32_t *)nullptr, avg_out, \
	                   tile && !coop ? L.d_cls : (uint8_t *)nullptr, L.far_ring, L.far_thr10, tile && !coop ? L.d_cls_stat : (unsigned long long *)nullptr, \
	                   coop ? 0u : c16_bound,                      \
	                   (!coop && tile && q24_ring(L, skip, want_gen, gs1, tab)) ? 1 : 0, SEGN, WS)
		if (seg) MM2C_WS(true, dim3((unsigned)L.n_tasks, (unsigned)((L.longest_task + PREPASS_SEG - 1) / PREPASS_SEG)), PREPASS_SEG, L.d_seg_ws);
		else MM2C_WS(false, dim3((unsigned)L.n_tasks), 0, (unsigned long long *)nullptr);
#undef MM2C_WS
	}
	hipError_t e = hipGetLastError();
	if (n_launches && !no_prepass) ++*n_launches;
	if (e == hipSuccess && tile && !coop && L.d_cls && L.d_cls_stat && (L.far_ring == 1 || c16_bound != 0)) {
		hipLaunchKernelGGL(chain_cls_settle, dim3((unsigned)((L.n_tasks + 255) / 256)), dim3(256), 0, st, L.n_tasks, L.d_cls, L.d_cls_stat, L.far_ring == 1 ? 1 : 0,
		                   c16_bound != 0 ? L.wide_pct : 100);
		e = hipGetLastError();
		if (n_launches) ++*n_launches;
	}
	if (e == hipSuccess && L.cut.max_pieces > 0) {
		hipLaunchKernelGGL(chain_cut, dim3((unsigned)L.n_tasks), dim3(64), 0, st, L.cut.seg_min, L.n_tasks, L.d_offsets, L.d_order,
		                   (const uint4 *)L.d_anchors, d_avg, L.d_st, L.cut, tile ? (const uint8_t *)L.d_cls : (const uint8_t *)nullptr);
		e = hipGetLastError();
		if (n_launches) ++*n_launches;
	}
	if (e == hipSuccess && coop_auto) {
		hipLaunchKernelGGL(chain_route, dim3(1), dim3(256), 0, st, L.cut);
		e = hipGetLastError();
		if (n_launches) ++*n_launches;
	}
	if (e == hipSuccess && ev_dp_begin) e = hipEventRecord(ev_dp_begin, st);
	LaunchArgs L1 = L; L1.d_avg = d_avg;
	for (int pass = 0; pass < 2 && e == hipSuccess; ++pass) {
		const bool gen = want_gen || pass == 1;
		if (pass == 1 && (want_gen || (P.flags & KF_IGNORE_SEG))) break;
		const int flagged = pass;
		if (pass == 1) { L.cut.d_live = nullptr; L1.cut.d_live = nullptr; }
		if (coop && !gen) { e = launch_coop(L, d_avg, st, tab, flagged, n_launches); continue; }
		if (coop_auto && !gen) e = launch_coop(L, d_avg, st, tab, flagged, n_launches);
		if (tile && (!gen || tile_gen)) { e = launch_tile(L, d_avg, st, skip, gen, gs1, far_, tab, flagged, n_launches); if (n_launches) ++*n_launches; continue; }
// ... 19 lines not shown
```

### minimap2-fpga_amd/csrc/mm2chain_api.cpp

```cpp
#include "api_internal.h"
#include "mm2chain_split.h"
#include <string>
#include <cctype>
#include <pthread.h>
#include <sched.h>

namespace mm2c_api {

thread_local char g_err[512] = "";

int fail(int code, const char *fmt, ...)
{
	va_list ap;
	va_start(ap, fmt);
	vsnprintf(g_err, sizeof(g_err), fmt, ap);
	va_end(ap);
	return code;
}

Global G;
StageStats SS;

static std::mutex g_async_mu;
static std::thread *g_async_th = nullptr;
// ... 388 lines not shown
{
	if (const int rc = check_offsets(n_tasks, off)) return rc;
	order.resize((size_t)n_tasks);
	std::iota(order.begin(), order.end(), 0);
	std::stable_sort(order.begin(), order.end(), [&](int32_t x, int32_t y) { return off[x + 1] - off[x] > off[y + 1] - off[y]; });
	return 0;
}


size_t layout_epilogue(mm2c::EpiArgs &E, char *base, size_t tot, size_t nt, size_t sort_tmp)
{
	size_t at = 0;
	auto take = [&](size_t bytes) { const size_t o = at; at = (at + bytes + 255) & ~(size_t)255; return base + o; };
	E.key0 = (uint64_t *)take(tot * 8); E.key1 = (uint64_t *)take(tot * 8); E.u2 = (uint64_t *)take(tot * 8); E.rkey1 = (uint64_t *)take(tot * 8);
	E.v = (int32_t *)take(tot * 4); E.own = (int32_t *)take(tot * 4); E.ctop = (int32_t *)take(tot * 4); E.rk2kk = (int32_t *)take(tot * 4);
	E.dest = (int32_t *)take(tot * 4); E.val0 = (int32_t *)take(tot * 4); E.val1 = (int32_t *)take(tot * 4);
	E.seg_begin = (uint32_t *)take(nt * 4); E.seg_end1 = (uint32_t *)take(nt * 4); E.seg_end2 = (uint32_t *)take(nt * 4);
	E.cnt_u = (int32_t *)take(nt * 4); E.cnt_b = (int32_t *)take(nt * 4);
	E.sort_tmp = take(sort_tmp ? sort_tmp : 1); E.sort_tmp_bytes = sort_tmp;
	return at;
}

int epilogue_debug_phases() { const char *dbg = getenv("MM2C_EPI_PHASES"); return dbg ? atoi(dbg) : 0; }

}

using namespace mm2c_api;

struct mm2c_plan {
	mm2c_params_t par;
	int device = 0;
	const int64_t *d_off_user = nullptr;
	int64_t n_tasks = 0, total = 0;
	int64_t *d_off = nullptr; int32_t *d_order = nullptr, *d_status = nullptr, *d_t = nullptr, *d_st = nullptr; float *d_avg_ws = nullptr; uint8_t *d_cls = nullptr;
	unsigned long long *d_seg_ws = nullptr;
	hipEvent_t ev_pre = nullptr, ev0 = nullptr, ev1 = nullptr, ev_e0 = nullptr, ev_e1 = nullptr;
	mm2c_api::AuxSet aux;
	bool ran = false, epi_ran = false;
	mm2c::LaunchInfo info = {};
	std::vector<int32_t> sizes_desc;
	char *d_cut = nullptr;
	mm2c::CutArgs cut;
	char *d_epi = nullptr;
	mm2c::EpiArgs E;
};

extern "C" {

const char *mm2c_last_error(void) { return g_err; }

int mm2c_init(int device_ordinal)
{
	async_init_join();
	std::lock_guard<std::mutex> lk(G.mu);
	if (G.ready) return 0;
	{
		const char *q = getenv("GPU_MAX_HW_QUEUES");
		static bool told = false;
		if (!q && !told && getenv("MM2C_QUIET") == nullptr) {
			told = true;
			fprintf(stderr, "[mm2chain] GPU_MAX_HW_QUEUES is %s: the upload / compute streams of the host-batch pipelines may share a hardware queue "
			                "(export GPU_MAX_HW_QUEUES=2 before the process's first HIP call)\n", "unset (runtime default 4)");
		}
	}
	int n_dev = 0;
	hipError_t e = hipGetDeviceCount(&n_dev);
	if (e != hipSuccess || n_dev <= 0)
// ... 318 lines not shown
		if (value < 0 || value > 6) return fail(MM2C_E_ARG, "pipeline_taper must be 0 .. 6");
		G.pipeline_taper = value;
		return 0;
	}
	if (strcmp(key, "pipeline_min_chunk") == 0) {
		if (value < 1024) return fail(MM2C_E_ARG, "pipeline_min_chunk must be >= 1024");
		G.pipeline_min_chunk = value;
		return 0;
	}
	if (strcmp(key, "coop_waves") == 0) {
		if (value < 0 || value > 64) return fail(MM2C_E_ARG, "coop_waves must be 0 .. 64 (0 / 1: one wave per task always; any other value: the cooperative kernel, which is built for 16 waves per task)");
		G.coop_waves = value;
		return 0;
	}
	if (strcmp(key, "combine_max_anchors") == 0) {
		if (value < 0) return fail(MM2C_E_ARG, "combine_max_anchors must be >= 0");
		G.combine_max_anchors = (size_t)value;
		return 0;
	}
	if (strcmp(key, "combiner_lanes") == 0) {
		if (value < 1 || value > 16) return fail(MM2C_E_ARG, "combiner_lanes must be 1 .. 16");
		G.combiner_lanes = value;
		return 0;
	}
	if (strcmp(key, "pipe_coop_chunks") == 0) {
		if (value < 0) return fail(MM2C_E_ARG, "pipe_coop_chunks must be >= 0");
		G.pipe_coop_chunks = value;
		return 0;
	}
	if (strcmp(key, "q24_ring") == 0) {
		G.q24_ring = value != 0;
		return 0;
	}
	if (strcmp(key, "pin_workers") == 0) {
		G.pin_workers = value != 0;
		return 0;
	}
	if (strcmp(key, "decline_when_busy") == 0) {
		if (value < 0 || value > 2) return fail(MM2C_E_ARG, "decline_when_busy must be 0 (never decline), 1 (by the slot's measured service time) or 2 (round 5's rule: booked predictions)");
		G.decline_when_busy = value;
		return 0;
	}
	if (strcmp(key, "direct_pass") == 0) {
		G.direct_pass = value != 0;
		return 0;
	}
	if (strcmp(key, "coop_plans") == 0) {
		if (value < 0 || value > 2) return fail(MM2C_E_ARG, "coop_plans must be 0 (never), 1 (every plan of at most coop_max_tasks tasks) or 2 (per run: few long pieces)");
		G.coop_plans = value;
		return 0;
	}
	if (strcmp(key, "host_st") == 0) {
		G.host_st = value != 0;
		return 0;
	}
	if (strcmp(key, "fused_out") == 0) {
		G.fused_out = value != 0;
		return 0;
	}
	if (strcmp(key, "single_launch") == 0) { G.single_launch = value != 0; return MM2C_OK; }
	if (strcmp(key, "fuse_st") == 0) { G.fuse_st = value != 0; return MM2C_OK; }
	if (strcmp(key, "seg_prepass") == 0) { G.seg_prepass = value != 0; return MM2C_OK; }
	if (strcmp(key, "coop_w8_above") == 0) {
		if (value < 0) return fail(MM2C_E_ARG, "coop_w8_above must be >= 0 (pieces beyond which the cooperative kernel takes eight waves per piece instead of sixteen)");
		G.coop_w8_above = (int)std::min<int64_t>(value, 1 << 30);
		return MM2C_OK;
// ... 93 lines not shown
	if (e == hipSuccess) e = dev_alloc((void **)&pl->d_order, nt * 4);
	if (e == hipSuccess) e = dev_alloc((void **)&pl->d_status, nt * 4);
	if (e == hipSuccess) e = dev_alloc((void **)&pl->d_t, tot * 4);
	if (e == hipSuccess) e = dev_alloc((void **)&pl->d_st, tot * 4);
	if (e == hipSuccess) e = dev_alloc((void **)&pl->d_avg_ws, nt * 4);
	if (e == hipSuccess) e = dev_alloc((void **)&pl->d_cls, ((nt + 15) & ~(size_t)15) + 32 * mm2c::CLS_STAT_SLOTS);
	if (e == hipSuccess && n_tasks > 0 && pl->sizes_desc[0] >= 65536) {
		e = dev_alloc((void **)&pl->d_seg_ws, nt * 32);
		if (e == hipSuccess) e = hipMemset(pl->d_seg_ws, 0, nt * 32);
	}
	if (e == hipSuccess && n_tasks > 0) {
		std::vector<int64_t> off((size_t)n_tasks + 1);
		for (int64_t k = 0; k <= n_tasks; ++k) off[(size_t)k] = h_offsets[k] - h_offsets[0];
		e = hipMemcpy(pl->d_off, off.data(), ((size_t)n_tasks + 1) * 8, hipMemcpyHostToDevice);
		if (e == hipSuccess) e = hipMemcpy(pl->d_order, order.data(), (size_t)n_tasks * 4, hipMemcpyHostToDevice);
	}
	if (e == hipSuccess) e = hipEventCreate(&pl->ev_pre);
	if (e == hipSuccess) e = hipEventCreate(&pl->ev0);
	if (e == hipSuccess) e = hipEventCreate(&pl->ev1);
	if (e != hipSuccess) {
		fail(MM2C_E_HIP, "mm2c_plan_create: %s", hipGetErrorString(e));
		mm2c_plan_destroy(pl);
		return nullptr;
	}
	return pl;
}

static void plan_destroy_impl(mm2c_plan_t *pl, bool wait)
{
	if (!pl) return;
	{
		DeviceScope on(pl->device);
		if (wait && (pl->ran || pl->epi_ran)) { ScopedNs timed(SS.free_ns); (void)hipDeviceSynchronize(); }
		dev_free_synced(pl->d_off); dev_free_synced(pl->d_order); dev_free_synced(pl->d_status); dev_free_synced(pl->d_t); dev_free_synced(pl->d_st);
		dev_free_synced(pl->d_avg_ws); dev_free_synced(pl->d_seg_ws); dev_free_synced(pl->d_cls); dev_free_synced(pl->d_epi); dev_free_synced(pl->d_cut);
		if (pl->ev_pre) (void)hipEventDestroy(pl->ev_pre);
		if (pl->ev0) (void)hipEventDestroy(pl->ev0); if (pl->ev1) (void)hipEventDestroy(pl->ev1);
		if (pl->ev_e0) (void)hipEventDestroy(pl->ev_e0); if (pl->ev_e1) (void)hipEventDestroy(pl->ev_e1);
		aux_release(pl->aux);
	}
	delete pl;
}

void mm2c_plan_destroy(mm2c_plan_t *pl) { plan_destroy_impl(pl, true); }

int64_t mm2c_plan_total_anchors(const mm2c_plan_t *pl) { return pl ? pl->total : 0; }

int mm2c_plan_set_device_offsets(mm2c_plan_t *pl, const int64_t *d_offsets)
{
	if (!pl) return fail(MM2C_E_ARG, "plan is NULL");
	pl->d_off_user = d_offsets;
	return 0;
}

int mm2c_plan_run_device(mm2c_plan_t *pl, const void *d_anchors, const float *d_avg_qspan, int32_t *d_f, int32_t *d_p, void *stream)
{
	if (!pl) return fail(MM2C_E_ARG, "plan is NULL");
	if (!lib_ready()) return fail_not_ready();
	if (pl->n_tasks == 0 || pl->total == 0) return 0;
	if (!d_anchors || !d_f || !d_p) return fail(MM2C_E_ARG, "device pointer is NULL");
	DeviceScope on(pl->device);
	HIP_TRY(on.err);
	hipStream_t st;
	if (const int rc = resolve_stream(stream, pl->device, &st)) return rc;
	mm2c::LaunchArgs L;
	L.P = to_kparams(&pl->par);
	L.n_tasks = pl->n_tasks; L.d_offsets = pl->d_off_user ? pl->d_off_user : pl->d_off; L.d_order = pl->d_order;
	L.d_anchors = d_anchors; L.d_avg = d_avg_qspan; L.d_pbase = nullptr; L.d_f = d_f; L.d_p = d_p; L.d_t = pl->d_t; L.d_st = pl->d_st; L.d_status = pl->d_status;
	L.d_avg_ws = pl->d_avg_ws;
	L.d_cls = pl->d_cls; L.far_ring = G.far_ring; L.far_thr10 = G.far_thr10;
	L.d_cls_stat = (unsigned long long *)(pl->d_cls + (((size_t)std::max<int64_t>(pl->n_tasks, 1) + 15) & ~(size_t)15));
	HIP_TRY(hipMemsetAsync(L.d_cls_stat, 0, 32 * mm2c::CLS_STAT_SLOTS, st));
	L.ring_class = G.ring_class; L.force_tab = G.force_tab; L.compact = G.compact_ring; L.q24 = G.q24_ring; L.wide_pct = G.wide_pct; L.noskip_loop = G.noskip_loop;
	HIP_TRY(hipMemsetAsync(pl->d_status, 0, (size_t)pl->n_tasks * 4, st));
	const int coop_mode = G.coop_waves.load() > 1 ? G.coop_plans.load() : 0;
	const int64_t longest = pl->sizes_desc.empty() ? 0 : (int64_t)pl->sizes_desc[0];
	const bool will_cut = G.plan_cut && G.seg_min > 0 && longest >= G.plan_cut_min;
	if (pl->d_seg_ws && !pl->d_off_user && G.seg_prepass.load()) { L.d_seg_ws = pl->d_seg_ws; L.longest_task = longest; }
	L.coop_waves = 0; L.coop_w8_above = G.coop_w8_above.load(); L.fuse_st = G.fuse_st.load();
	if (coop_mode == 1 && pl->n_tasks <= G.coop_max_tasks) L.coop_waves = G.coop_waves.load();
	else if (coop_mode == 2 && !will_cut && !pl->d_off_user && mm2c::coop_pays(pl->n_tasks, longest, pl->total, G.coop_w8_above.load())) L.coop_waves = G.coop_waves.load();
	else if (coop_mode == 2 && will_cut) L.coop_waves = -1;
	if (L.coop_waves > 1) L.max_task_anchors = longest;
	if (L.coop_waves <= 1 && G.plan_cut && G.seg_min > 0) {
		const int seg_min = (pl->n_tasks <= mm2c::COOP_ROUTE_MAX_PIECES && longest >= 65536) ? (int)std::max<int64_t>(G.seg_min, longest / 64) : (int)G.seg_min;
		int64_t extra = 0;
		for (size_t k = 0; k < pl->sizes_desc.size() && pl->sizes_desc[k] >= G.plan_cut_min; ++k) extra += pl->sizes_desc[k] / seg_min;
		const int64_t max_pieces = pl->n_tasks + extra;
		if (extra > 0 && max_pieces <= (int64_t)INT32_MAX) {
			if (!pl->d_cut || pl->cut.max_pieces != max_pieces || pl->cut.seg_min != seg_min) {
				dev_free(pl->d_cut); pl->d_cut = nullptr;
				const size_t mp = (size_t)max_pieces;
				size_t at = 0;
				auto take = [&](size_t bytes) { const size_t o = at; at = (at + bytes + 255) & ~(size_t)255; return o; };
				const size_t o_cnt = take(4), o_stat = take(mp * 4), o_hc = take((size_t)pl->n_tasks * 4), o_start = take(mp * 8), o_end = take(mp * 8),
				             o_pb = take(mp * 4), o_avg = take(mp * 4), o_cls = take(mp);
				HIP_TRY(dev_alloc((void **)&pl->d_cut, at));
				char *b = pl->d_cut;
				pl->cut.max_pieces = max_pieces; pl->cut.seg_min = seg_min;
				pl->cut.d_count = (int32_t *)(b + o_cnt); pl->cut.d_status = (int32_t *)(b + o_stat); pl->cut.d_has_cut = (int32_t *)(b + o_hc);
				pl->cut.d_start = (int64_t *)(b + o_start); pl->cut.d_end = (int64_t *)(b + o_end);
// ... 32 lines not shown
	HIP_TRY(mm2c::launch_predict(pl->par.max_dist_x, pl->n_tasks, pl->d_off_user ? pl->d_off_user : pl->d_off, pl->d_order, d_anchors, d_num_subparts,
	                             d_total_subparts, d_total_trip_count, st));
	G.launches += 1;
	return 0;
}

int mm2c_plan_last_prepass_ms(mm2c_plan_t *pl, float *ms)
{
	if (!pl || !ms) return fail(MM2C_E_ARG, "NULL argument");
	if (!pl->ran) return fail(MM2C_E_ARG, "plan has not been run");
	HIP_TRY(hipEventSynchronize(pl->ev0));
	HIP_TRY(hipEventElapsedTime(ms, pl->ev_pre, pl->ev0));
	return 0;
}

int mm2c_plan_run_device_n(mm2c_plan_t *pl, const void *d_anchors, int64_t n_anchors, const float *d_avg_qspan, int64_t n_avg,
                           int32_t *d_f, int64_t n_f, int32_t *d_p, int64_t n_p, void *stream)
{
	if (!pl) return fail(MM2C_E_ARG, "plan is NULL");
	if (n_anchors < pl->total || n_f < pl->total || n_p < pl->total || (d_avg_qspan && n_avg < pl->n_tasks))
		return fail(MM2C_E_TOOBIG, "a buffer is shorter than the plan's %lld anchors / %lld tasks (anchors %lld, f %lld, p %lld, avg %lld)",
		            (long long)pl->total, (long long)pl->n_tasks, (long long)n_anchors, (long long)n_f, (long long)n_p, (long long)n_avg);
	return mm2c_plan_run_device(pl, d_anchors, d_avg_qspan, d_f, d_p, stream);
}

int mm2c_plan_last_variant(mm2c_plan_t *pl, char *buf, size_t len)
{
	if (!pl || !buf || len == 0) return fail(MM2C_E_ARG, "NULL argument");
	if (!pl->ran) return fail(MM2C_E_ARG, "plan has not been run");
	format_variant(pl->info, buf, len);
	return 0;
}

int mm2c_plan_last_route(mm2c_plan_t *pl, int64_t *pieces, int64_t *one_wave_pieces, int64_t *coop_pieces)
{
	if (!pl || !pieces || !one_wave_pieces || !coop_pieces) return fail(MM2C_E_ARG, "NULL argument");
	if (!pl->ran) return fail(MM2C_E_ARG, "plan has not been run");
	if (pl->info.route_auto && pl->d_cut) {
		DeviceScope on(pl->device);
		HIP_TRY(on.err);
		HIP_TRY(hipEventSynchronize(pl->ev1));
		int32_t w[4] = {0, 0, 0, 0};
		HIP_TRY(hipMemcpy(w, pl->d_cut, sizeof(w), hipMemcpyDeviceToHost));
		*pieces = w[0]; *one_wave_pieces = w[1]; *coop_pieces = w[2] + w[3];
		return 0;
	}
	*pieces = pl->n_tasks;
	*one_wave_pieces = pl->info.coop ? 0 : pl->n_tasks; *coop_pieces = pl->info.coop ? pl->n_tasks : 0;
	if (pl->info.cut && pl->d_cut) {
		DeviceScope on(pl->device);
		HIP_TRY(on.err);
		HIP_TRY(hipEventSynchronize(pl->ev1));
		int32_t w = 0;
		HIP_TRY(hipMemcpy(&w, pl->d_cut, sizeof(w), hipMemcpyDeviceToHost));
		*pieces = w; *one_wave_pieces = w;
	}
	return 0;
}

int mm2c_route_pieces(int64_t pieces, int64_t longest, int64_t total) { const int w8 = G.coop_w8_above.load(); return mm2c::coop_pays(pieces, longest, total, w8) ? (pieces > w8 ? 8 : 16) : 1; }

int mm2c_plan_last_kernel_ms(mm2c_plan_t *pl, float *ms)
{
	if (!pl || !ms) return fail(MM2C_E_ARG, "NULL argument");
	if (!pl->ran) return fail(MM2C_E_ARG, "plan has not been run");
	HIP_TRY(hipEventSynchronize(pl->ev1));
// ... 82 lines not shown
```

### minimap2-fpga_amd/mm2chain/_native.py

```python
import ctypes as C
import os

_HERE = os.path.dirname(os.path.abspath(__file__))
LIB_PATH = os.environ.get("MM2C_LIB_PATH") or os.path.join(os.path.dirname(_HERE), "libmm2chain_hip.so")

MM2C_F_IGNORE_SEG = 0x1
MM2C_F_FORCE_GENERAL = 0x2


class Params(C.Structure):
    _fields_ = [("max_dist_x", C.c_int32), ("max_dist_y", C.c_int32), ("bw", C.c_int32),
                ("max_skip", C.c_int32), ("max_iter", C.c_int32), ("gap_scale", C.c_float),
                ("is_cdna", C.c_int32), ("n_segs", C.c_int32), ("q_span_override", C.c_int32),
                ("flags", C.c_int32)]


class Stream(C.Structure):
    _fields_ = [("par", Params), ("min_cnt", C.c_int32), ("min_sc", C.c_int32), ("n_tasks", C.c_int64), ("total", C.c_int64),
                ("offsets", C.POINTER(C.c_int64)), ("anchors", C.c_void_p)]


class Stats(C.Structure):
    _fields_ = [("tasks", C.c_uint64), ("anchors", C.c_uint64), ("launches", C.c_uint64), ("segments", C.c_uint64), ("host_call_ns", C.c_uint64), ("passes", C.c_uint64)]

# ... 26 lines not shown


class IndexStats(C.Structure):
    _fields_ = [(k, C.c_uint64) for k in ("calls", "chunks", "bases", "minimizers", "keys", "h2d_ns", "sketch_ns", "sort_ns", "group_ns", "occ_ns", "replicate_ns")]


C_SYMBOLS = {
    "mm2c_init": (C.c_int, [C.c_int]),
    "mm2c_init_devices": (C.c_int, [C.c_int, C.POINTER(C.c_int)]),
    "mm2c_init_async": (C.c_int, [C.c_int]),
    "mm2c_init_wait": (C.c_int, []),
    "mm2c_warm_up": (C.c_int, []),
    "mm2c_device_count": (C.c_int, []),
    "mm2c_numa_cpulist": (C.c_int, [C.c_char_p, C.c_char_p, C.c_char_p, C.c_size_t]),
    "mm2c_slot_worker_node": (C.c_int, [C.c_int]),
    "mm2c_split_tasks": (C.c_int, [C.c_int64, C.c_void_p, C.c_int, C.c_void_p]),
    "mm2c_shutdown": (None, []),
    "mm2c_last_error": (C.c_char_p, []),
    "mm2c_device_info": (C.c_int, [C.c_char_p, C.c_size_t, C.POINTER(C.c_int), C.POINTER(C.c_size_t)]),
    "mm2c_device_identity": (C.c_int, [C.POINTER(C.c_int), C.c_char_p, C.c_size_t, C.c_char_p, C.c_size_t]),
    "mm2c_tune": (C.c_int, [C.c_char_p, C.c_int]),
    "mm2c_split_model": (C.c_int, [C.c_char_p] + [C.POINTER(C.c_float)] * 5),
    "mm2c_params_map_ont": (None, [C.POINTER(Params)]),
    "mm2c_params_fpga_v2": (None, [C.POINTER(Params), C.c_int32, C.c_int32, C.c_int32, C.c_int32]),
    "mm2c_plan_create": (C.c_void_p, [C.POINTER(Params), C.c_int64, C.c_void_p]),
    "mm2c_plan_destroy": (None, [C.c_void_p]),
    "mm2c_plan_total_anchors": (C.c_int64, [C.c_void_p]),
    "mm2c_plan_run_device": (C.c_int, [C.c_void_p, C.c_void_p, C.c_void_p, C.c_void_p, C.c_void_p, C.c_void_p]),
    "mm2c_plan_set_device_offsets": (C.c_int, [C.c_void_p, C.c_void_p]),
    "mm2c_plan_run_device_n": (C.c_int, [C.c_void_p, C.c_void_p, C.c_int64, C.c_void_p, C.c_int64, C.c_void_p, C.c_int64, C.c_void_p, C.c_int64, C.c_void_p]),
    "mm2c_plan_predict_device": (C.c_int, [C.c_void_p, C.c_void_p, C.c_void_p, C.c_void_p, C.c_void_p, C.c_void_p]),
    "mm2c_plan_last_kernel_ms": (C.c_int, [C.c_void_p, C.POINTER(C.c_float)]),
    "mm2c_plan_last_variant": (C.c_int, [C.c_void_p, C.c_char_p, C.c_size_t]),
    "mm2c_plan_last_route": (C.c_int, [C.c_void_p, C.POINTER(C.c_int64), C.POINTER(C.c_int64), C.POINTER(C.c_int64)]),
    "mm2c_route_pieces": (C.c_int, [C.c_int64, C.c_int64, C.c_int64]),
    "mm2c_last_host_variant": (C.c_int, [C.c_char_p, C.c_size_t]),
    "mm2c_debug_label_hits": (C.c_int, [C.POINTER(C.c_ulonglong), C.c_int]),
    "mm2c_plan_last_prepass_ms": (C.c_int, [C.c_void_p, C.POINTER(C.c_float)]),
    "mm2c_chain_batch_host": (C.c_int, [C.POINTER(Params), C.c_int64, C.c_void_p, C.c_void_p, C.c_void_p, C.c_void_p, C.c_void_p]),
    "mm2c_pinned_alloc": (C.c_void_p, [C.c_size_t]),
    "mm2c_pinned_free": (None, [C.c_void_p]),
    "mm2c_chain_task_host": (C.c_int, [C.POINTER(Params), C.c_int64, C.c_void_p, C.c_float, C.c_void_p, C.c_void_p, C.c_int]),
    "mm2c_chain_task_host_pred": (C.c_int, [C.POINTER(Params), C.c_int64, C.c_void_p, C.c_float, C.c_void_p, C.c_void_p, C.c_int, C.c_float, C.c_float]),
    "mm2c_get_slot_stats": (C.c_int, [C.c_int, C.POINTER(SlotStats)]),
    "mm2c_route_slot": (C.c_int, [C.c_int, C.c_void_p, C.c_int]),
    "mm_chain_dp": (C.c_void_p, [C.c_int, C.c_int, C.c_int, C.c_int, C.c_int, C.c_int, C.c_int, C.c_float, C.c_int, C.c_int,
                                 C.c_int64, C.c_void_p, C.POINTER(C.c_int), C.POINTER(C.c_void_p), C.c_void_p, C.c_int]),
    "mm2c_plan_chains_device": (C.c_int, [C.c_void_p, C.c_void_p, C.c_void_p, C.c_void_p, C.c_int, C.c_int, C.c_void_p, C.c_void_p,
                                          C.c_void_p, C.c_void_p, C.c_void_p]),
    "mm2c_plan_chains_device_n": (C.c_int, [C.c_void_p, C.c_void_p, C.c_int64, C.c_void_p, C.c_int64, C.c_void_p, C.c_int64, C.c_int, C.c_int,
                                            C.c_void_p, C.c_int64, C.c_void_p, C.c_int64, C.c_void_p, C.c_int64, C.c_void_p, C.c_int64, C.c_void_p]),
    "mm2c_plan_last_epilogue_ms": (C.c_int, [C.c_void_p, C.POINTER(C.c_float)]),
    "mm2c_chain_epilogue_host": (C.c_int, [C.c_int, C.c_int, C.c_int64, C.c_void_p, C.c_void_p, C.c_void_p, C.c_void_p, C.c_int,
                                           C.c_void_p, C.c_void_p, C.c_void_p, C.c_void_p]),
    "mm2c_mm_chain_dp_batch_host": (C.c_int, [C.POINTER(Params), C.c_int, C.c_int, C.c_int64, C.c_void_p, C.c_void_p, C.c_int,
                                              C.c_void_p, C.c_void_p, C.c_void_p, C.c_void_p]),
    "mm2c_seedplan_create": (C.c_void_p, [C.c_int64, C.c_void_p, C.c_void_p]),
    "mm2c_seedplan_destroy": (None, [C.c_void_p]),
    "mm2c_seedplan_run_device": (C.c_int, [C.c_void_p, C.c_void_p, C.c_void_p, C.c_void_p, C.c_void_p, C.c_void_p]),
    "mm2c_seedplan_run_device_n": (C.c_int, [C.c_void_p, C.c_void_p, C.c_int64, C.c_void_p, C.c_int64, C.c_void_p, C.c_int64, C.c_void_p, C.c_int64,
                                             C.c_void_p]),
    "mm2c_seedplan_run_device_skip": (C.c_int, [C.c_void_p, C.c_void_p, C.c_int64, C.c_void_p, C.c_int64, C.c_void_p, C.c_int64, C.c_void_p, C.c_void_p,
                                                C.c_int64, C.c_void_p, C.c_void_p]),
    "mm2c_seedplan_set_heap_sort": (C.c_int, [C.c_void_p, C.c_int]),
    "mm2c_seedplan_check": (C.c_int, [C.c_void_p, C.POINTER(C.c_int64)]),
    "mm2c_seedplan_last_ms": (C.c_int, [C.c_void_p, C.POINTER(C.c_float)]),
# ... 91 lines not shown
```

### minimap2-fpga_amd/mm2chain/batch.py

```python
import ctypes as C
import os
import numpy as np
import torch

from . import _native as N
from .params import Params

_inited = False


def init(device=None):
    global _inited
    lib = N.load()
    if device is None:
        device = torch.cuda.current_device() if torch.cuda.is_available() and not os.environ.get("MM2C_DEVICES") else -1
    N.check(lib.mm2c_init(int(device)), "mm2c_init")
    _inited = True


def init_devices(ordinals):
    global _inited
    arr = (C.c_int * len(ordinals))(*[int(d) for d in ordinals])
    N.check(N.load().mm2c_init_devices(len(ordinals), arr), "mm2c_init_devices")
    _inited = True
# ... 93 lines not shown

    def chains(self, anchors: torch.Tensor, f: torch.Tensor, p: torch.Tensor, min_cnt: int, min_sc: int, stream=None):
        assert anchors.is_cuda and anchors.dtype == torch.int64 and f.dtype == torch.int32 and p.dtype == torch.int32
        dev = anchors.device
        u_off = torch.empty(self.n_tasks + 1, dtype=torch.int64, device=dev)
        b_off = torch.empty(self.n_tasks + 1, dtype=torch.int64, device=dev)
        u = torch.empty(max(self.total, 1), dtype=torch.int64, device=dev)
        b = torch.empty((max(self.total, 1), 2), dtype=torch.int64, device=dev)
        st = stream if stream is not None else torch.cuda.current_stream().cuda_stream
        N.check(self.lib.mm2c_plan_chains_device_n(self.handle, anchors.data_ptr(), anchors.numel() // 2, f.data_ptr(), f.numel(), p.data_ptr(), p.numel(),
                                                   min_cnt, min_sc, u_off.data_ptr(), u_off.numel(), u.data_ptr(), u.numel(), b_off.data_ptr(),
                                                   b_off.numel(), b.data_ptr(), b.numel() // 2, st), "mm2c_plan_chains_device_n")
        return u_off, u, b_off, b

    def last_epilogue_ms(self):
        ms = C.c_float(0)
        N.check(self.lib.mm2c_plan_last_epilogue_ms(self.handle, C.byref(ms)), "mm2c_plan_last_epilogue_ms")
        return ms.value

    def last_kernel_ms(self):
        ms = C.c_float(0)
        N.check(self.lib.mm2c_plan_last_kernel_ms(self.handle, C.byref(ms)), "mm2c_plan_last_kernel_ms")
        return ms.value

    def last_route(self):
        a, b, c = C.c_int64(0), C.c_int64(0), C.c_int64(0)
        N.check(self.lib.mm2c_plan_last_route(self.handle, C.byref(a), C.byref(b), C.byref(c)), "mm2c_plan_last_route")
        return int(a.value), int(b.value), int(c.value)

    def last_variant(self):
        buf = C.create_string_buffer(192)
        N.check(self.lib.mm2c_plan_last_variant(self.handle, buf, len(buf)), "mm2c_plan_last_variant")
        return buf.value.decode()

    def last_prepass_ms(self):
        ms = C.c_float(0)
        N.check(self.lib.mm2c_plan_last_prepass_ms(self.handle, C.byref(ms)), "mm2c_plan_last_prepass_ms")
        return ms.value

    def close(self):
        if self.handle:
            self.lib.mm2c_plan_destroy(self.handle)
            self.handle = None

    def __del__(self):
        try:
            self.close()
        except Exception:
            pass


class PinnedArray:

    def __init__(self, shape, dtype):
        self.lib = N.load()
        self.nbytes = int(np.prod(shape)) * np.dtype(dtype).itemsize
        self.ptr = self.lib.mm2c_pinned_alloc(self.nbytes)
        if not self.ptr:
            N.check(-1, "mm2c_pinned_alloc")
        buf = (C.c_char * max(self.nbytes, 1)).from_address(self.ptr)
        self.array = np.frombuffer(buf, dtype=dtype, count=int(np.prod(shape))).reshape(shape)

    def __del__(self):
        try:
            if self.ptr:
                self.array = None
# ... 605 lines not shown
```

Measured before the change: 7.398 billion anchors/s.

## Pack f and p into one 32-bit word for the compact-ring tile kernel

```diff
diff --git a/include/mm2chain.h b/include/mm2chain.h
--- a/include/mm2chain.h
+++ b/include/mm2chain.h
@@ -69,6 +69,7 @@
 int mm2c_plan_last_route(mm2c_plan_t *plan, int64_t *pieces, int64_t *one_wave_pieces, int64_t *coop_pieces);
 int mm2c_route_pieces(int64_t pieces, int64_t longest, int64_t total);
 int mm2c_plan_last_variant(mm2c_plan_t *plan, char *buf, size_t len);
+int mm2c_plan_last_classes(mm2c_plan_t *plan, unsigned char *cls, int64_t n);
 int  mm2c_last_host_variant(char *buf, size_t len);
 int  mm2c_debug_label_hits(unsigned long long *hits , int reset);
 int mm2c_plan_last_prepass_ms(mm2c_plan_t *plan, float *ms);
diff --git a/minimap2-fpga_amd/csrc/api_internal.h b/minimap2-fpga_amd/csrc/api_internal.h
--- a/minimap2-fpga_amd/csrc/api_internal.h
+++ b/minimap2-fpga_amd/csrc/api_internal.h
@@ -40,6 +40,7 @@
 	std::atomic<int> wide_pct{40};
 	std::atomic<int> split_streams{1};
 	std::atomic<int> compact_ring{1};
+	std::atomic<int> packed_fp{1};
 	std::atomic<int> q24_ring{1};
 	std::atomic<int> force_tab{0};
 	std::atomic<int> far_ring{1};
@@ -156,8 +157,8 @@
 {
 	if (I.tile && I.coop) snprintf(buf, len, "chain_dp_coop<W=%d,NX=%d,NF=%d,GS1=%d,FAR=%d,TAB=%d> loop=%s classes=0 cut=0 compact=0 coop=%d st=%s", I.coop, I.nx, I.nf, I.gs1,
 	                               I.far_, I.tab, I.asm_loop ? "asm" : "c++", I.coop, I.fused_st ? "kernel" : "prepass");
-	else if (I.tile) snprintf(buf, len, "chain_dp_tile<NX=%d,NF=%d,SKIP=%d,GEN=%d,GS1=%d,FAR=%d,TAB=%d> loop=%s classes=%d cut=%d compact=%d q24=%d", I.nx, I.nf, I.skip, I.gen, I.gs1,
-	                     I.far_, I.tab, I.asm_loop ? "asm" : "c++", I.classes, I.cut, I.c16, I.q24);
+	else if (I.tile) snprintf(buf, len, "chain_dp_tile<NX=%d,NF=%d,SKIP=%d,GEN=%d,GS1=%d,FAR=%d,TAB=%d> loop=%s classes=%d cut=%d compact=%d q24=%d packed_fp=%d", I.nx, I.nf, I.skip, I.gen, I.gs1,
+	                     I.far_, I.tab, I.asm_loop ? "asm" : "c++", I.classes, I.cut, I.c16, I.q24, I.packed);
 	else snprintf(buf, len, "chain_dp_wave<R=%d,SKIP=%d,GEN=%d,GS1=%d,FAR=%d> loop=c++ classes=0 cut=%d", I.r, I.skip, I.gen, I.gs1, I.far_, I.cut);
 }
 void note_host_variant(const mm2c::LaunchInfo &I);
diff --git a/minimap2-fpga_amd/csrc/chain_dp_coop.h b/minimap2-fpga_amd/csrc/chain_dp_coop.h
--- a/minimap2-fpga_amd/csrc/chain_dp_coop.h
+++ b/minimap2-fpga_amd/csrc/chain_dp_coop.h
@@ -592,7 +592,7 @@
 				flush(k);
 				int k2 = k;
 				if (ASM) {
-#define MM2C_CALL(FN, LO0) FN<NX, NF>(i0, __builtin_amdgcn_readfirstlane(k), cnt, P.max_skip, avg, f, p, pbase, a, t, own_x, tx1_l, own_q, tq1_l, span_l, lo_c, \
+#define MM2C_CALL(FN, LO0) FN<NX, NF>(i0, __builtin_amdgcn_readfirstlane(k), cnt, P.max_skip, avg, f, p, f, pbase, a, t, own_x, tx1_l, own_q, tq1_l, span_l, lo_c, \
                                  LO0, tw_l, own_f, own_p, addr0, addr0b, lomc_v, ownst, rl, mdqbw_v, X.bw_v, sent_v, 0, 0 MM2C_LC_ARG)
 #ifdef MM2C_LABEL_COUNT
 					int lc_v = 0;
diff --git a/minimap2-fpga_amd/csrc/chain_dp_tile.h b/minimap2-fpga_amd/csrc/chain_dp_tile.h
--- a/minimap2-fpga_amd/csrc/chain_dp_tile.h
+++ b/minimap2-fpga_amd/csrc/chain_dp_tile.h
@@ -39,15 +39,22 @@
 struct Lds {
 	static constexpr int SN = 64 * NX;
 	static constexpr int XS = RING ? 4 : 8;
+	static constexpr int FS = RING == 3 ? 4 : 8;
 	static constexpr int TILE = 64 * XS;
 	static constexpr int RB = SN * XS;
-	static constexpr int XQ = 0, FP = RB, ST = FP + NF * 512, QH = ST + SN, GAP = QH + (RING == 2 ? SN : 0),
+	static constexpr int XQ = 0, FP = RB, ST = FP + NF * 64 * FS, QH = ST + SN, GAP = QH + (RING == 2 ? SN : 0),
 	                     G = GAP + (TAB ? 1024 : 0), BYTES = G + (GEN ? NX * 64 : 0);
-	static constexpr int FMASK = NF * 512 - 1;
+	static constexpr int FMASK = NF * 64 * FS - 1;
 	static constexpr int SBITS = __builtin_ctz(SN);
 };
 
+constexpr int PK_FBITS = 18;
+constexpr int PK_MAX_F = (1 << (PK_FBITS - 1)) - 1;
 constexpr int FBIAS = 14;
+
+__device__ __forceinline__ int pack_fp(int f_biased, int p) { return (int)(((unsigned)p << PK_FBITS) | ((unsigned)f_biased & ((1u << PK_FBITS) - 1))); }
+__device__ __forceinline__ int packed_f(int w) { return (int)((unsigned)w << (32 - PK_FBITS)) >> (32 - PK_FBITS); }
+__device__ __forceinline__ int packed_p(int w) { return w >> PK_FBITS; }
 
 struct AnchorCtx {
 	int xi1, qi1;
@@ -63,6 +70,7 @@
 struct TileMem {
 	char *lds;
 	const uint4 *a; const int32_t *f, *p; int32_t *t;
+	const int32_t *w;
 	int pbase;
 };
 
@@ -115,7 +123,12 @@
 template <class LY, int NF>
 __device__ __forceinline__ void ring_fp(const TileMem &M, int addr, int depth, int base, int rl, int &fj, int &pj)
 {
-	if (depth <= NF) {
+	if (LY::FS == 4) {
+		int v;
+		if (depth <= NF) v = *(const int *)(M.lds + LY::FP + (addr & LY::FMASK));
+		else v = __hip_atomic_load(&M.w[max(base + rl, 0)], __ATOMIC_RELAXED, __HIP_MEMORY_SCOPE_WORKGROUP);
+		fj = packed_f(v) + FBIAS; pj = packed_p(v);
+	} else if (depth <= NF) {
 		const int o = (LY::XS == 4 ? addr << 1 : addr) & LY::FMASK;
 		const int2 fp = *(const int2 *)(M.lds + LY::FP + o);
 		fj = fp.x + FBIAS; pj = fp.y;
@@ -279,6 +292,13 @@
 	"v_perm_b32 %[u1], " MM2C_R_Q ", " MM2C_R_X ", %[selq]\n\t" "v_sub_u32 %[dq], %[qi1], %[u1]\n\t"
 #define MM2C_OLDADDR_W "v_add_u32 %[vb], 0x400, %[addr]\n\t"
 #define MM2C_OLDADDR_C "v_add_lshl_u32 %[vb], %[addr], %[c200], 1\n\t"
+#define MM2C_OLDADDR_P "v_add_u32 %[vb], 0x200, %[addr]\n\t"
+#define MM2C_RDFP_8 "ds_read_b64 " MM2C_R_FP ", %[u2] offset:%[FPOFF]\n\t"
+#define MM2C_RDFP_4 "ds_read_b32 " MM2C_R_F ", %[u2] offset:%[FPOFF]\n\t"
+#define MM2C_UNPACK_8 ""
+#define MM2C_UNPACK_4 "v_ashrrev_i32 " MM2C_R_P ", %[FBITS], " MM2C_R_F "\n\t" "v_bfe_i32 " MM2C_R_F ", " MM2C_R_F ", 0, %[FBITS]\n\t"
+#define MM2C_FGFIX_8 "v_subrev_u32 " MM2C_R_P ", %[pbase], " MM2C_R_P "\n\t" "v_max_i32 " MM2C_R_P ", -1, " MM2C_R_P "\n\t" "v_add_u32 " MM2C_R_F ", -14, " MM2C_R_F "\n\t"
+#define MM2C_FGFIX_4 MM2C_UNPACK_4
 #define MM2C_FAR_REQ "v_add_u32 %[u2], %[fb], %[rl]\n\t" "v_max_i32 %[u2], 0, %[u2]\n\t" "v_lshlrev_b32 %[u2], 4, %[u2]\n\t" \
 	"global_load_dword %[fx], %[u2], %[aptr]\n\t" "global_load_dword %[fq], %[u2], %[aptr] offset:8\n\t" "s_sub_i32 %[fb], %[fb], 64\n\t"
 #define MM2C_SCORE_CMP "v_or_b32 %[va], 1, %[dd]\n\t" "v_ffbh_u32 %[va], %[va]\n\t" "v_lshrrev_b32 %[va], 1, %[va]\n\t" "v_cvt_f32_u32 %[vc], %[dd]\n\t" \
@@ -476,6 +496,15 @@
 	"global_load_dword " MM2C_R_F ", %[u2], %[fptr] sc0\n\t" \
 	SCORE \
 	"s_waitcnt vmcnt(0)\n\t"
+#define MM2C_FG_PACKED(SCORE) \
+	"s_lshl_b32 %[t0], %[d], 6\n\t" \
+	"s_sub_i32 %[base], %[i0], %[t0]\n\t" \
+	"v_add_u32 %[u2], %[base], %[rl]\n\t" \
+	"v_max_i32 %[u2], 0, %[u2]\n\t" \
+	"v_lshlrev_b32 %[u2], 2, %[u2]\n\t" \
+	"global_load_dword " MM2C_R_F ", %[u2], %[wptr] sc0\n\t" \
+	SCORE \
+	"s_waitcnt vmcnt(0)\n\t"
 #if MM2C_DEEP_PREFETCH
 #define MM2C_FG_W(SCORE) \
 	"s_lshl_b32 %[t0], %[d], 6\n\t" \
@@ -554,9 +583,9 @@
 #define MM2C_LB_FOLD "0x10000000"
 #define MM2C_LB_DONE "0x20000000"
 #define MM2C_LB_SPEC "0x40000000"
-#define MM2C_SCAN_TILE_ASM(NAME, TABV, C16V, XQ1, NEXT_XQ, RFILTER, OLDADDR, BACK, OWNFILTER, FARFILTER, RDXQ, SEG_FG, CLOB, SCORE, ADDF, SEG_RD, SEG_LK, SEG_HF, SEG_TAIL, SEG_END, SEG_DONE, LNEXT) \
+#define MM2C_SCAN_TILE_ASM(NAME, TABV, C16V, XQ1, NEXT_XQ, RFILTER, OLDADDR, BACK, OWNFILTER, FARFILTER, RDXQ, SEG_FG, CLOB, RDFP, UNPACK, FGFIX, STSH, SCORE, ADDF, SEG_RD, SEG_LK, SEG_HF, SEG_TAIL, SEG_END, SEG_DONE, LNEXT) \
 template <int NX, int NF> \
-__device__ __forceinline__ int NAME(int i0, int k_start, int cnt, int max_skip, float avg, const int32_t *f, const int32_t *p, int pbase, const uint4 *a, \
+__device__ __forceinline__ int NAME(int i0, int k_start, int cnt, int max_skip, float avg, const int32_t *f, const int32_t *p, const int32_t *wq, int pbase, const uint4 *a, \
                                     int32_t *tg, int tx, int tx1, int tq, int tq1, int tspan, int tlo, int tlo0, int tw, int &own_f, int &own_p, \
                                     int addr1, int addr2, int lomc, int ownst, int rl, int mdqbw_v, int bw_v, int sent_v, int addr1q, int selq_v MM2C_LC_PARAM) \
 { \
@@ -619,12 +648,14 @@
 		MM2C_LC(MM2C_LB_OLD) \
 		OLDADDR                                         \
 		"v_and_b32 %[u2], %[FMASK], %[vb]\n\t"           \
-		"v_bfe_u32 %[vb], %[vb], 3, %[SBITS]\n\t"        \
+		"v_bfe_u32 %[vb], %[vb], " STSH ", %[SBITS]\n\t"    \
 		"s_cmp_gt_u32 %[d], %[NFI]\n\t" \
 		"s_cbranch_scc1 Lfg_%=\n\t" \
-		"ds_read_b64 " MM2C_R_FP ", %[u2] offset:%[FPOFF]\n\t" \
+		RDFP \
 		SCORE \
-		"s_waitcnt lgkmcnt(0)\n" \
+		"s_waitcnt lgkmcnt(0)\n\t" \
+		UNPACK \
+		"\n" \
 		"Lhf_%=:\n\t" \
 		MM2C_LC(MM2C_LB_HF) \
 		SEG_HF \
@@ -641,9 +672,7 @@
 		"Lfg_%=:\n\t" \
 		MM2C_LC(MM2C_LB_FG) \
 		SEG_FG(SCORE) \
-		"v_subrev_u32 " MM2C_R_P ", %[pbase], " MM2C_R_P "\n\t" \
-		"v_max_i32 " MM2C_R_P ", -1, " MM2C_R_P "\n\t" \
-		"v_add_u32 " MM2C_R_F ", -14, " MM2C_R_F "\n\t" \
+		FGFIX \
 		"s_branch Lhf_%=\n" \
 		"Lpart_%=:\n\t" \
 		MM2C_LC(MM2C_LB_PART) \
@@ -836,18 +865,19 @@
 		  [dr] "=&v"(dr), [dq] "=&v"(dq), [dd] "=&v"(dd), [u1] "=&v"(u1), [u2] "=&v"(u2), \
 		  [sc] "=&v"(sc), [va] "=&v"(va), [vb] "=&v"(vb), [vc] "=&v"(vc), [addr] "=&v"(addr), [s16v] "=&v"(s16v), [lom1v] "=&v"(lom1v), [fx] "=&v"(fx), [fq] "=&v"(fq), \
 		  [own_f] "+v"(own_f), [own_p] "+v"(own_p) MM2C_PROBE_OPERAND MM2C_LC_OPERAND \
-		: [i0] "s"(i0), [kstart] "s"(k_start), [cnt] "s"(cnt), [icnt1] "s"(i0 + cnt + 1), [i063] "s"(i0 + 63), [c200] "s"(0x200), [maxskip] "s"(max_skip), [avg] "s"(avg), [fptr] "s"(f), [pptr] "s"(p), [pbase] "s"(pbase), [aptr] "s"(a), [tptr] "s"(tg), \
+		: [i0] "s"(i0), [kstart] "s"(k_start), [cnt] "s"(cnt), [icnt1] "s"(i0 + cnt + 1), [i063] "s"(i0 + 63), [c200] "s"(0x200), [maxskip] "s"(max_skip), [avg] "s"(avg), [fptr] "s"(f), [pptr] "s"(p), [wptr] "s"(wq), [pbase] "s"(pbase), [aptr] "s"(a), [tptr] "s"(tg), \
 		  [tx] "v"(tx), [tx1] "v"(tx1), [tq] "v"(tq), [tq1] "v"(tq1), [tspan] "v"(tspan), [tlo] "v"(tlo), [tlo0] "v"(tlo0), [tw] "v"(tw), \
 		  [addr1] "v"(addr1), [addr2] "v"(addr2), [lomc] "v"(lomc), [ownst] "v"(ownst), [rl] "v"(rl), [mdqbw] "v"(mdqbw_v), [bw] "v"(bw_v), [sent] "v"(sent_v), \
 		  [addr1q] "v"(addr1q), [selq] "v"(selq_v), [QHOFF] "n"(LY::QH), \
 		  [XQOFF] "n"(LY::XQ), [FPOFF] "n"(LY::FP), [STOFF] "n"(LY::ST), [RBM1] "n"(LY::RB - 1), [FMASK] "n"(LY::FMASK), \
-		  [SNM1] "n"(LY::SN - 1), [RMASK] "n"(64 * NX - 1), [SBITS] "n"(LY::SBITS), [NFI] "n"(NF), [GAPOFF] "n"(LYT::GAP), [NXM1] "n"(NX - 1), [REACH] "n"(64 * NX) \
+		  [SNM1] "n"(LY::SN - 1), [RMASK] "n"(64 * NX - 1), [SBITS] "n"(LY::SBITS), [NFI] "n"(NF), [GAPOFF] "n"(LYT::GAP), [NXM1] "n"(NX - 1), [REACH] "n"(64 * NX), [FBITS] "n"(PK_FBITS) \
 		: "memory", "vcc", "scc", MM2C_R_X, MM2C_R_Q, MM2C_R_F, MM2C_R_P MM2C_FG_CLOB(CLOB)); \
 	return cnt + c; \
 }
 
-#define MM2C_RING_W MM2C_XQ1_W, MM2C_NEXT_XQ_W, MM2C_RFILTER_W, MM2C_OLDADDR_W, MM2C_BACK_W, MM2C_OWNFILTER_W, MM2C_FARFILTER_W, MM2C_RDXQ_W, MM2C_FG_W, PF2
-#define MM2C_RING_C MM2C_XQ1_C, MM2C_NEXT_XQ_C, MM2C_RFILTER_C, MM2C_OLDADDR_C, MM2C_BACK_C, MM2C_OWNFILTER_C, MM2C_FARFILTER_C, MM2C_RDXQ_C, MM2C_FG_PLAIN, PF0
+#define MM2C_RING_W MM2C_XQ1_W, MM2C_NEXT_XQ_W, MM2C_RFILTER_W, MM2C_OLDADDR_W, MM2C_BACK_W, MM2C_OWNFILTER_W, MM2C_FARFILTER_W, MM2C_RDXQ_W, MM2C_FG_W, PF2, MM2C_RDFP_8, MM2C_UNPACK_8, MM2C_FGFIX_8, "3"
+#define MM2C_RING_C MM2C_XQ1_C, MM2C_NEXT_XQ_C, MM2C_RFILTER_C, MM2C_OLDADDR_C, MM2C_BACK_C, MM2C_OWNFILTER_C, MM2C_FARFILTER_C, MM2C_RDXQ_C, MM2C_FG_PLAIN, PF0, MM2C_RDFP_8, MM2C_UNPACK_8, MM2C_FGFIX_8, "3"
+#define MM2C_RING_P MM2C_XQ1_C, MM2C_NEXT_XQ_C, MM2C_RFILTER_C, MM2C_OLDADDR_P, MM2C_BACK_C, MM2C_OWNFILTER_C, MM2C_FARFILTER_C, MM2C_RDXQ_C, MM2C_FG_PACKED, PF0, MM2C_RDFP_4, MM2C_UNPACK_4, MM2C_FGFIX_4, "2"
 #define MM2C_SCAN_TILE_ASM_(...) MM2C_SCAN_TILE_ASM(__VA_ARGS__)
 #define MM2C_LEAN MM2C_RD_LEAN, MM2C_LK_LEAN, MM2C_HF_LEAN, MM2C_TAIL_LEAN, MM2C_END_LEAN, "", "Lloop_%="
 #define MM2C_FARS MM2C_RD_FAR, MM2C_LK_FAR, MM2C_HF_FAR, MM2C_TAIL_FAR, MM2C_END_FAR, MM2C_DONE_FAR, "Lret_%="
@@ -859,7 +889,11 @@
 MM2C_SCAN_TILE_ASM_(scan_tile_asm_tab_c, true, true, MM2C_RING_C, MM2C_SCORE_TAB, MM2C_ADDF_TAB, MM2C_LEAN)
 MM2C_SCAN_TILE_ASM_(scan_tile_asm_cmp_far_c, false, true, MM2C_RING_C, MM2C_SCORE_CMP, MM2C_ADDF_CMP, MM2C_FARS)
 MM2C_SCAN_TILE_ASM_(scan_tile_asm_tab_far_c, true, true, MM2C_RING_C, MM2C_SCORE_TAB, MM2C_ADDF_TAB, MM2C_FARS)
-#define MM2C_RING_Q MM2C_XQ1_Q, MM2C_NEXT_XQ_Q, MM2C_RFILTER_Q, MM2C_OLDADDR_C, MM2C_BACK_C, MM2C_OWNFILTER_W, MM2C_FARFILTER_W, MM2C_RDXQ_W, MM2C_FG_PLAIN, PF0
+MM2C_SCAN_TILE_ASM_(scan_tile_asm_cmp_p, false, 3, MM2C_RING_P, MM2C_SCORE_CMP, MM2C_ADDF_CMP, MM2C_LEAN)
+MM2C_SCAN_TILE_ASM_(scan_tile_asm_tab_p, true, 3, MM2C_RING_P, MM2C_SCORE_TAB, MM2C_ADDF_TAB, MM2C_LEAN)
+MM2C_SCAN_TILE_ASM_(scan_tile_asm_cmp_far_p, false, 3, MM2C_RING_P, MM2C_SCORE_CMP, MM2C_ADDF_CMP, MM2C_FARS)
+MM2C_SCAN_TILE_ASM_(scan_tile_asm_tab_far_p, true, 3, MM2C_RING_P, MM2C_SCORE_TAB, MM2C_ADDF_TAB, MM2C_FARS)
+#define MM2C_RING_Q MM2C_XQ1_Q, MM2C_NEXT_XQ_Q, MM2C_RFILTER_Q, MM2C_OLDADDR_C, MM2C_BACK_C, MM2C_OWNFILTER_W, MM2C_FARFILTER_W, MM2C_RDXQ_W, MM2C_FG_PLAIN, PF0, MM2C_RDFP_8, MM2C_UNPACK_8, MM2C_FGFIX_8, "3"
 MM2C_SCAN_TILE_ASM_(scan_tile_asm_cmp_q, false, 2, MM2C_RING_Q, MM2C_SCORE_CMP, MM2C_ADDF_CMP, MM2C_LEAN)
 MM2C_SCAN_TILE_ASM_(scan_tile_asm_tab_q, true, 2, MM2C_RING_Q, MM2C_SCORE_TAB, MM2C_ADDF_TAB, MM2C_LEAN)
 MM2C_SCAN_TILE_ASM_(scan_tile_asm_cmp_far_q, false, 2, MM2C_RING_Q, MM2C_SCORE_CMP, MM2C_ADDF_CMP, MM2C_FARS)
@@ -869,13 +903,13 @@
 #ifdef MM2C_LABEL_COUNT
 #define MM2C_WAVES_PER_SIMD(C16V, BYTES) 1
 #else
-#define MM2C_WAVES_PER_SIMD(C16V, BYTES) ((C16V) == 1 && (BYTES) <= 6144 ? 7 : (C16V) == 2 && (BYTES) <= 7424 ? 6 : 1)
+#define MM2C_WAVES_PER_SIMD(C16V, BYTES) (((C16V) == 1 || (C16V) == 3) && (BYTES) <= 6144 ? 7 : (C16V) == 2 && (BYTES) <= 7424 ? 6 : 1)
 #endif
 __global__ void __launch_bounds__(64, MM2C_WAVES_PER_SIMD(C16, (Lds<NX, NF, GEN, TAB, C16>::BYTES)))
 chain_dp_tile(KParams P, int64_t n_tasks, const int64_t *__restrict__ offsets, const int32_t *__restrict__ order,
               const uint4 *__restrict__ a_all, const float *__restrict__ avg_in, const int32_t *__restrict__ pbase_in,
               const int32_t *__restrict__ st_all, int32_t *__restrict__ f_all, int32_t *__restrict__ p_all, int32_t *__restrict__ t_all,
-              int32_t *__restrict__ status, int only_flagged, const int64_t *__restrict__ ends, const int32_t *__restrict__ n_live,
+              int32_t *__restrict__ w_all , int32_t *__restrict__ status, int only_flagged, const int64_t *__restrict__ ends, const int32_t *__restrict__ n_live,
               const uint8_t *__restrict__ cls, int my_cls, int cls_mask)
 {
 	static_assert(!C16 || (SKIP && !GEN && (GS1 || TAB)), "the compact and the q24 ring belong to the variants of the hand-written loop");
@@ -900,6 +934,7 @@
 	const uint4 *a = a_all + base0;
 	const int32_t *st = st_all + base0;
 	int32_t *f = f_all + base0, *p = p_all + base0, *t = FAR ? t_all + base0 : nullptr;
+	int32_t *w = C16 == 3 ? w_all + base0 : f;
 	if (ASMV && (uint32_t)(uintptr_t)(void *)lds != 0) { if (lane == 0) status[task] = 3; return; }
 
 	const int pbase = pbase_in ? pbase_in[task] : 0;
@@ -932,7 +967,7 @@
 	asm volatile("" : "+v"(X.mdq1_v), "+v"(X.bw_v), "+v"(sent_v), "+v"(mdqbw_v));
 	if (C16 == 2) asm volatile("" : "+v"(selq_v));
 	TileMem M;
-	M.lds = lds; M.a = a; M.f = f; M.p = p; M.t = t; M.pbase = pbase;
+	M.lds = lds; M.a = a; M.f = f; M.p = p; M.t = t; M.w = w; M.pbase = pbase;
 
 	int own_x = 0, own_q = 0, own_g = 0, own_f = 0, own_p = -1;
 	int seg0 = 0;
@@ -1005,15 +1040,18 @@
 
 		for (int k = 0; k < cnt; ++k) {
 			if (ASM) {
-#define MM2C_CALL(FN, LO0) FN<NX, NF>(i0, __builtin_amdgcn_readfirstlane(k), cnt, P.max_skip, avg, f, p, pbase, a, t, own_x, tx1_l, own_q, tq1_l, span_l, lo_c, \
+#define MM2C_CALL(FN, LO0) FN<NX, NF>(i0, __builtin_amdgcn_readfirstlane(k), cnt, P.max_skip, avg, f, p, w, pbase, a, t, own_x, tx1_l, own_q, tq1_l, span_l, lo_c, \
                                  LO0, tw_l, own_f, own_p, addr0, addr0b, lomc_v, ownst, rl, mdqbw_v, X.bw_v, sent_v, addr0 >> 2, selq_v MM2C_LC_ARG)
 				if (C16 == 2) {
 					if (FAR && tile_far) k = TAB ? MM2C_CALL(scan_tile_asm_tab_far_q, lo_l) : MM2C_CALL(scan_tile_asm_cmp_far_q, lo_l);
 					else k = TAB ? MM2C_CALL(scan_tile_asm_tab_q, lo_l) : MM2C_CALL(scan_tile_asm_cmp_q, lo_l);
 				} else if (C16) {
-#define MM2C_CALLC(FN, LO0) FN<NX, NF>(i0, __builtin_amdgcn_readfirstlane(k), cnt, P.max_skip, avg, f, p, pbase, a, t, own_xq, own_xq1, own_xq, own_xq1, span_l, lo_c, \
+#define MM2C_CALLC(FN, LO0) FN<NX, NF>(i0, __builtin_amdgcn_readfirstlane(k), cnt, P.max_skip, avg, f, p, w, pbase, a, t, own_xq, own_xq1, own_xq, own_xq1, span_l, lo_c, \
                                  LO0, tw_l, own_f, own_p, addr0, addr0b, lomc_v, ownst, rl, mdqbw_v, X.bw_v, sent_v, 0, 0 MM2C_LC_ARG)
-					if (FAR && tile_far) k = TAB ? MM2C_CALLC(scan_tile_asm_tab_far_c, lo_l) : MM2C_CALLC(scan_tile_asm_cmp_far_c, lo_l);
+					if (C16 == 3) {
+						if (FAR && tile_far) k = TAB ? MM2C_CALLC(scan_tile_asm_tab_far_p, lo_l) : MM2C_CALLC(scan_tile_asm_cmp_far_p, lo_l);
+						else k = TAB ? MM2C_CALLC(scan_tile_asm_tab_p, lo_l) : MM2C_CALLC(scan_tile_asm_cmp_p, lo_l);
+					} else if (FAR && tile_far) k = TAB ? MM2C_CALLC(scan_tile_asm_tab_far_c, lo_l) : MM2C_CALLC(scan_tile_asm_cmp_far_c, lo_l);
 					else k = TAB ? MM2C_CALLC(scan_tile_asm_tab_c, lo_l) : MM2C_CALLC(scan_tile_asm_cmp_c, lo_l);
 #undef MM2C_CALLC
 				} else if (FAR && tile_far) k = TAB ? MM2C_CALL(scan_tile_asm_tab_far, lo_l) : MM2C_CALL(scan_tile_asm_cmp_far, lo_l);
@@ -1021,7 +1059,7 @@
 #undef MM2C_CALL
 #ifdef MM2C_LABEL_COUNT
 				{
-					const int row = (C16 == 1 ? 4 : 0) | (TAB ? 2 : 0) | ((FAR && tile_far) ? 1 : 0);
+					const int row = (C16 == 1 || C16 == 3 ? 4 : 0) | (TAB ? 2 : 0) | ((FAR && tile_far) ? 1 : 0);
 					if (lane < 32 && lc_v != 0) atomicAdd(&g_label_hits[row * 32 + lane], (unsigned long long)(unsigned)lc_v);
 					lc_v = 0;
 				}
@@ -1053,7 +1091,11 @@
 			write_lane2(own_f, own_p, __builtin_amdgcn_readfirstlane(c.best), __builtin_amdgcn_readfirstlane(c.best_j), L);
 		}
 		if (rl < cnt) { f[idx] = own_f; p[idx] = own_p < 0 ? own_p : own_p + pbase; }
-		{
+		if (LY::FS == 4) {
+			const int v = pack_fp(own_f - FBIAS, own_p);
+			*(int *)(lds + LY::FP + ((idx << 2) & LY::FMASK)) = v;
+			if (rl < cnt) w[idx] = v;
+		} else {
 			const int o = (idx << 3) & LY::FMASK;
 			*(int2 *)(lds + LY::FP + o) = make_int2(own_f - FBIAS, own_p);
 		}
diff --git a/minimap2-fpga_amd/csrc/chain_kernel.h b/minimap2-fpga_amd/csrc/chain_kernel.h
--- a/minimap2-fpga_amd/csrc/chain_kernel.h
+++ b/minimap2-fpga_amd/csrc/chain_kernel.h
@@ -6,6 +6,7 @@
 namespace mm2c {
 
 enum { KF_IGNORE_SEG = 0x1, KF_FORCE_GENERAL = 0x2 };
+constexpr int PK_MAX_N = 8192;
 constexpr int CLS_STAT_SLOTS = 64;
 
 struct KParams {
@@ -45,6 +46,8 @@
 	int noskip_loop = 1;
 	int compact = 1;
 	int q24 = 1;
+	int packed_fp = 1;
+	int32_t *d_w = nullptr;
 	unsigned long long *d_cls_stat = nullptr;
 	int wide_pct = 40;
 	int far_thr10 = 7;
@@ -78,6 +81,7 @@
 	int classes;
 	int c16;
 	int q24;
+	int packed;
 	int cut;
 	int coop;
 	int host_out;
diff --git a/minimap2-fpga_amd/csrc/chain_kernel.hip b/minimap2-fpga_amd/csrc/chain_kernel.hip
--- a/minimap2-fpga_amd/csrc/chain_kernel.hip
+++ b/minimap2-fpga_amd/csrc/chain_kernel.hip
@@ -16,6 +16,9 @@
 #endif
 #ifndef MM2C_CNX
 #define MM2C_CNX 16
+#endif
+#ifndef MM2C_PNF
+#define MM2C_PNF 4
 #endif
 #ifndef MM2C_CNF
 #define MM2C_CNF 2
@@ -185,6 +188,7 @@
                    unsigned long long *__restrict__ cls_stat ,
                    unsigned q_span_max ,
                    int q24 ,
+                   int packed_fp ,
                    int seg_anchors, unsigned long long *__restrict__ seg_ws)
 {
 	const int lane = threadIdx.x;
@@ -277,19 +281,25 @@
 		if (!s_last) return;
 		far_sum = 0; span_sum = 0; q_min = s_qmin; q_max = s_qmax;
 	}
+	if ((cls_out || avg_out) && n > 0) {
+		for (int o = 32; o > 0; o >>= 1) span_sum += __shfl_xor(span_sum, o);
+		if ((lane & 63) == 0 && span_sum) atomicAdd(&s_sum, (unsigned long long)span_sum);
+	}
 	if (cls_out && n > 0) {
 		for (int o = 32; o > 0; o >>= 1) { q_min = min(q_min, __shfl_xor(q_min, o)); q_max = max(q_max, __shfl_xor(q_max, o)); }
 		if ((lane & 63) == 0) { atomicMin(&s_qmin, q_min); atomicMax(&s_qmax, q_max); }
 		__syncthreads();
 		const int wide = (q_span_max == 0 || (unsigned)s_qmax - (unsigned)s_qmin > q_span_max) ? 2 : 0;
 		const int huge = (q24 && (s_qmin < 0 || s_qmax >= (1 << 24))) ? 4 : 0;
+		const unsigned long long f_bound = P.span_override >= 0 ? (unsigned long long)P.span_override * (unsigned long long)n : s_sum;
+		const int fits = (packed_fp && n <= PK_MAX_N && f_bound <= (unsigned long long)PK_MAX_F) ? 8 : 0;
 		if (far_ring == 1) {
 			for (int o = 32; o > 0; o >>= 1) far_sum += __shfl_xor(far_sum, o);
 			if ((lane & 63) == 0 && far_sum) atomicAdd(&s_far, (unsigned long long)far_sum);
 			__syncthreads();
 			if (lane == 0) {
 				const int c = (!huge && n >= 1024 && 10 * s_far > (unsigned long long)far_thr10 * (unsigned long long)n) ? 1 : 0;
-				cls_out[task] = (uint8_t)(c | wide | huge);
+				cls_out[task] = (uint8_t)(c | wide | huge | fits);
 				if (cls_stat) {
 					unsigned long long *cs = cls_stat + 4 * (task & (CLS_STAT_SLOTS - 1));
 					atomicAdd(&cs[1], (unsigned long long)n); if (c) atomicAdd(&cs[0], (unsigned long long)n);
@@ -297,13 +307,11 @@
 				}
 			}
 		} else if (lane == 0) {
-			cls_out[task] = (uint8_t)((far_ring == 2 && !huge ? 1 : 0) | wide | huge);
+			cls_out[task] = (uint8_t)((far_ring == 2 && !huge ? 1 : 0) | wide | huge | fits);
 			if (cls_stat) { unsigned long long *cs = cls_stat + 4 * (task & (CLS_STAT_SLOTS - 1)); atomicAdd(&cs[1], (unsigned long long)n); if (wide) atomicAdd(&cs[3], (unsigned long long)n); }
 		}
 	}
 	if (avg_out && n > 0) {
-		for (int o = 32; o > 0; o >>= 1) span_sum += __shfl_xor(span_sum, o);
-		if ((lane & 63) == 0) atomicAdd(&s_sum, (unsigned long long)span_sum);
 		__syncthreads();
 		if (lane == 0) avg_out[task] = (float)(__dmul_rn(.01, (double)(float)s_sum) / (double)n);
 	}
@@ -381,7 +389,7 @@
 	int c = cls[t];
 	if (all_wide) c |= 2;
 	if (settle_ring) {
-		if (4 * far < all) c &= 6;
+		if (4 * far < all) c &= ~1;
 		else if (4 * far > 3 * all && !(c & 4)) c |= 1;
 	}
 	cls[t] = (uint8_t)c;
@@ -607,12 +615,12 @@
 	if (L.cut.max_pieces > 0) {
 		hipLaunchKernelGGL((chain_dp_tile<NX, NF, SKIP, GEN, GS1, FAR, TAB, C16>), dim3((unsigned)L.cut.max_pieces), dim3(64), 0, st,
 		                   L.P, L.cut.max_pieces, L.cut.d_start, (const int32_t *)nullptr, (const uint4 *)L.d_anchors, L.cut.d_avg, L.cut.d_pbase, L.d_st, L.d_f, L.d_p,
-		                   L.d_t, L.cut.d_status, only_flagged, L.cut.d_end, L.cut.d_live ? L.cut.d_live : L.cut.d_count, with_cls ? (const uint8_t *)L.cut.d_cls : (const uint8_t *)nullptr, my_cls, cls_mask);
+		                   L.d_t, L.d_w, L.cut.d_status, only_flagged, L.cut.d_end, L.cut.d_live ? L.cut.d_live : L.cut.d_count, with_cls ? (const uint8_t *)L.cut.d_cls : (const uint8_t *)nullptr, my_cls, cls_mask);
 		return hipGetLastError();
 	}
 	hipLaunchKernelGGL((chain_dp_tile<NX, NF, SKIP, GEN, GS1, FAR, TAB, C16>), dim3((unsigned)L.n_tasks), dim3(64), 0, st,
 	                   L.P, L.n_tasks, L.d_offsets, L.d_order, (const uint4 *)L.d_anchors, d_avg, L.d_pbase, L.d_st, L.d_f, L.d_p, L.d_t,
-	                   L.d_status, only_flagged, (const int64_t *)nullptr, (const int32_t *)nullptr, with_cls ? (const uint8_t *)L.d_cls : (const uint8_t *)nullptr, my_cls, cls_mask);
+	                   L.d_w, L.d_status, only_flagged, (const int64_t *)nullptr, (const int32_t *)nullptr, with_cls ? (const uint8_t *)L.d_cls : (const uint8_t *)nullptr, my_cls, cls_mask);
 	return hipGetLastError();
 }
 
@@ -624,6 +632,8 @@
 	if (!L.compact || !asm_loop || !have_cls(L) || P.max_dist_x < 0 || P.max_dist_x > 65535 || P.max_dq < 1 || P.max_dq > 32768) return 0;
 	return 65535u - (unsigned)P.max_dq;
 }
+
+static bool packed_fp_ring(const LaunchArgs &L, bool asm_loop) { return L.packed_fp != 0 && L.d_w != nullptr && compact_q_span(L, asm_loop) != 0; }
 
 static bool q24_ring(const LaunchArgs &L, bool skip, bool gen, bool gs1, bool tab)
 {
@@ -651,10 +661,18 @@
 			if (!done) e = launch_tile_nx<2 * MM2C_NX, MM2C_NF1, SKIP, GEN, GS1, FAR, TAB, 0>(L, d_avg, sw, only_flagged, true, wide | 1, mask);
 			if (n_launches) ++*n_launches;
 		}
+	bool pk = false;
+	if constexpr (SKIP && !GEN && (GS1 || TAB)) pk = c16 && packed_fp_ring(L, true);
+	if constexpr (SKIP && !GEN && (GS1 || TAB))
+		if (e == hipSuccess && c16 && pk) { e = launch_tile_nx<MM2C_CNX, MM2C_CNF, SKIP, GEN, GS1, FAR, TAB, 1>(L, d_avg, sw, only_flagged, true, 0, 2 | 8); if (n_launches) ++*n_launches; }
 	bool joined = false;
 	if (forked) joined = hipEventRecord(L.ev_join, sw) == hipSuccess;
 	if constexpr (SKIP && !GEN && (GS1 || TAB))
-		if (e == hipSuccess && c16) { e = launch_tile_nx<MM2C_CNX, MM2C_CNF, SKIP, GEN, GS1, FAR, TAB, 1>(L, d_avg, st, only_flagged, true, 0, 2); if (n_launches) ++*n_launches; }
+		if (e == hipSuccess && c16) {
+			if (pk) e = launch_tile_nx<MM2C_CNX, MM2C_PNF, SKIP, GEN, GS1, FAR, TAB, 3>(L, d_avg, st, only_flagged, true, 8, 2 | 8);
+			else e = launch_tile_nx<MM2C_CNX, MM2C_CNF, SKIP, GEN, GS1, FAR, TAB, 1>(L, d_avg, st, only_flagged, true, 0, 2);
+			if (n_launches) ++*n_launches;
+		}
 	if (forked) {
 		const hipError_t ej = joined ? hipStreamWaitEvent(st, L.ev_join, 0) : hipStreamSynchronize(sw);
 		if (e == hipSuccess) e = joined ? ej : hipErrorUnknown;
@@ -807,8 +825,9 @@
 		info->classes = t0 && use_classes(L, skip, want_gen);
 		info->c16 = t0 && compact_q_span(L, info->asm_loop != 0) != 0;
 		info->q24 = t0 && info->classes && q24_ring(L, skip, want_gen, gs1, tab);
+		info->packed = t0 && info->c16 && packed_fp_ring(L, info->asm_loop != 0);
 		info->cut = L.cut.max_pieces > 0;
-		if (coop) { info->nx = COOP_NX; info->nf = COOP_NF; info->r = 64 * (COOP_NX - 1); info->far_ = (int64_t)P.max_iter > 64 * (COOP_NX - 1); info->classes = 0; info->c16 = 0; info->q24 = 0; }
+		if (coop) { info->nx = COOP_NX; info->nf = COOP_NF; info->r = 64 * (COOP_NX - 1); info->far_ = (int64_t)P.max_iter > 64 * (COOP_NX - 1); info->classes = 0; info->c16 = 0; info->q24 = 0; info->packed = 0; }
 	}
 	if (L.dry_run) return hipSuccess;
 	float *avg_out = L.d_avg ? nullptr : L.d_avg_ws;
@@ -830,7 +849,7 @@
 	                   (const ulonglong2 *)L.d_anchors, L.d_st, L.cut.max_pieces > 0 ? L.cut.d_has_cut : (int32_t *)nullptr, avg_out, \
 	                   tile && !coop ? L.d_cls : (uint8_t *)nullptr, L.far_ring, L.far_thr10, tile && !coop ? L.d_cls_stat : (unsigned long long *)nullptr, \
 	                   coop ? 0u : c16_bound,                      \
-	                   (!coop && tile && q24_ring(L, skip, want_gen, gs1, tab)) ? 1 : 0, SEGN, WS)
+	                   (!coop && tile && q24_ring(L, skip, want_gen, gs1, tab)) ? 1 : 0, (!coop && c16_bound != 0 && L.packed_fp != 0 && L.d_w != nullptr) ? 1 : 0, SEGN, WS)
 		if (seg) MM2C_WS(true, dim3((unsigned)L.n_tasks, (unsigned)((L.longest_task + PREPASS_SEG - 1) / PREPASS_SEG)), PREPASS_SEG, L.d_seg_ws);
 		else MM2C_WS(false, dim3((unsigned)L.n_tasks), 0, (unsigned long long *)nullptr);
 #undef MM2C_WS
diff --git a/minimap2-fpga_amd/csrc/mm2chain_api.cpp b/minimap2-fpga_amd/csrc/mm2chain_api.cpp
--- a/minimap2-fpga_amd/csrc/mm2chain_api.cpp
+++ b/minimap2-fpga_amd/csrc/mm2chain_api.cpp
@@ -444,7 +444,7 @@
 	int device = 0;
 	const int64_t *d_off_user = nullptr;
 	int64_t n_tasks = 0, total = 0;
-	int64_t *d_off = nullptr; int32_t *d_order = nullptr, *d_status = nullptr, *d_t = nullptr, *d_st = nullptr; float *d_avg_ws = nullptr; uint8_t *d_cls = nullptr;
+	int64_t *d_off = nullptr; int32_t *d_order = nullptr, *d_status = nullptr, *d_t = nullptr, *d_st = nullptr, *d_w = nullptr; float *d_avg_ws = nullptr; uint8_t *d_cls = nullptr;
 	unsigned long long *d_seg_ws = nullptr;
 	hipEvent_t ev_pre = nullptr, ev0 = nullptr, ev1 = nullptr, ev_e0 = nullptr, ev_e1 = nullptr;
 	mm2c_api::AuxSet aux;
@@ -829,6 +829,11 @@
 		G.q24_ring = value != 0;
 		return 0;
 	}
+	if (strcmp(key, "packed_fp") == 0) {
+		if (value < 0 || value > 1) return fail(MM2C_E_ARG, "packed_fp must be 0 or 1");
+		G.packed_fp = value;
+		return 0;
+	}
 	if (strcmp(key, "pin_workers") == 0) {
 		G.pin_workers = value != 0;
 		return 0;
@@ -988,7 +993,7 @@
 	{
 		DeviceScope on(pl->device);
 		if (wait && (pl->ran || pl->epi_ran)) { ScopedNs timed(SS.free_ns); (void)hipDeviceSynchronize(); }
-		dev_free_synced(pl->d_off); dev_free_synced(pl->d_order); dev_free_synced(pl->d_status); dev_free_synced(pl->d_t); dev_free_synced(pl->d_st);
+		dev_free_synced(pl->d_off); dev_free_synced(pl->d_order); dev_free_synced(pl->d_status); dev_free_synced(pl->d_t); dev_free_synced(pl->d_st); dev_free_synced(pl->d_w);
 		dev_free_synced(pl->d_avg_ws); dev_free_synced(pl->d_seg_ws); dev_free_synced(pl->d_cls); dev_free_synced(pl->d_epi); dev_free_synced(pl->d_cut);
 		if (pl->ev_pre) (void)hipEventDestroy(pl->ev_pre);
 		if (pl->ev0) (void)hipEventDestroy(pl->ev0); if (pl->ev1) (void)hipEventDestroy(pl->ev1);
@@ -1021,8 +1026,11 @@
 	if (const int rc = resolve_stream(stream, pl->device, &st)) return rc;
 	mm2c::LaunchArgs L;
 	L.P = to_kparams(&pl->par);
+	const bool packed_ok = G.packed_fp && pl->sizes_desc[0] <= mm2c::PK_MAX_N;
+	if (!pl->d_w && packed_ok && G.compact_ring && L.P.max_dist_x >= 0 && L.P.max_dist_x <= 65535 && L.P.max_dq >= 1 && L.P.max_dq <= 32768)
+		if (dev_alloc((void **)&pl->d_w, (size_t)std::max<int64_t>(pl->total, 1) * 4) != hipSuccess) { pl->d_w = nullptr; (void)hipGetLastError(); }
 	L.n_tasks = pl->n_tasks; L.d_offsets = pl->d_off_user ? pl->d_off_user : pl->d_off; L.d_order = pl->d_order;
-	L.d_anchors = d_anchors; L.d_avg = d_avg_qspan; L.d_pbase = nullptr; L.d_f = d_f; L.d_p = d_p; L.d_t = pl->d_t; L.d_st = pl->d_st; L.d_status = pl->d_status;
+	L.d_anchors = d_anchors; L.d_avg = d_avg_qspan; L.d_pbase = nullptr; L.d_f = d_f; L.d_p = d_p; L.d_t = pl->d_t; L.d_st = pl->d_st; L.d_w = pl->d_w; L.packed_fp = packed_ok ? 1 : 0; L.d_status = pl->d_status;
 	L.d_avg_ws = pl->d_avg_ws;
 	L.d_cls = pl->d_cls; L.far_ring = G.far_ring; L.far_thr10 = G.far_thr10;
 	L.d_cls_stat = (unsigned long long *)(pl->d_cls + (((size_t)std::max<int64_t>(pl->n_tasks, 1) + 15) & ~(size_t)15));
@@ -1121,6 +1129,19 @@
 	return 0;
 }
 
+int mm2c_plan_last_classes(mm2c_plan_t *pl, unsigned char *cls, int64_t n)
+{
+	if (!pl || !cls) return fail(MM2C_E_ARG, "NULL argument");
+	if (!pl->ran) return fail(MM2C_E_ARG, "plan has not been run");
+	if (n != pl->n_tasks) return fail(MM2C_E_ARG, "one byte per task of the plan");
+	if (n == 0) return 0;
+	DeviceScope on(pl->device);
+	HIP_TRY(on.err);
+	HIP_TRY(hipEventSynchronize(pl->ev1));
+	HIP_TRY(hipMemcpy(cls, pl->d_cls, (size_t)n, hipMemcpyDeviceToHost));
+	return 0;
+}
+
 int mm2c_plan_last_route(mm2c_plan_t *pl, int64_t *pieces, int64_t *one_wave_pieces, int64_t *coop_pieces)
 {
 	if (!pl || !pieces || !one_wave_pieces || !coop_pieces) return fail(MM2C_E_ARG, "NULL argument");
diff --git a/minimap2-fpga_amd/mm2chain/_native.py b/minimap2-fpga_amd/mm2chain/_native.py
--- a/minimap2-fpga_amd/mm2chain/_native.py
+++ b/minimap2-fpga_amd/mm2chain/_native.py
@@ -82,6 +82,7 @@
     "mm2c_plan_predict_device": (C.c_int, [C.c_void_p, C.c_void_p, C.c_void_p, C.c_void_p, C.c_void_p, C.c_void_p]),
     "mm2c_plan_last_kernel_ms": (C.c_int, [C.c_void_p, C.POINTER(C.c_float)]),
     "mm2c_plan_last_variant": (C.c_int, [C.c_void_p, C.c_char_p, C.c_size_t]),
+    "mm2c_plan_last_classes": (C.c_int, [C.c_void_p, C.POINTER(C.c_ubyte), C.c_int64]),
     "mm2c_plan_last_route": (C.c_int, [C.c_void_p, C.POINTER(C.c_int64), C.POINTER(C.c_int64), C.POINTER(C.c_int64)]),
     "mm2c_route_pieces": (C.c_int, [C.c_int64, C.c_int64, C.c_int64]),
     "mm2c_last_host_variant": (C.c_int, [C.c_char_p, C.c_size_t]),
diff --git a/minimap2-fpga_amd/mm2chain/batch.py b/minimap2-fpga_amd/mm2chain/batch.py
--- a/minimap2-fpga_amd/mm2chain/batch.py
+++ b/minimap2-fpga_amd/mm2chain/batch.py
@@ -149,6 +149,11 @@
         buf = C.create_string_buffer(192)
         N.check(self.lib.mm2c_plan_last_variant(self.handle, buf, len(buf)), "mm2c_plan_last_variant")
         return buf.value.decode()
+
+    def last_classes(self):
+        buf = (C.c_ubyte * max(self.n_tasks, 1))()
+        N.check(self.lib.mm2c_plan_last_classes(self.handle, buf, self.n_tasks), "mm2c_plan_last_classes")
+        return bytes(buf)[:self.n_tasks]
 
     def last_prepass_ms(self):
         ms = C.c_float(0)
```

Measured after the change: 7.620 billion anchors/s (median of 6 runs). 1.03x the previous value.
